# Superjomn/TiPS

Measured on AMD Instinct MI355X. Metric: device-resident fp32 bucket-sum GiB/s (% HBM peak); allreduce GiB/s 1/2/4/8 GPU, higher is better.
Workload: dtype f32

## Files before the change

### tips_amd/csrc/neg_protocol.cc

```cpp
#include "neg_protocol.h"

namespace tips {
namespace rt {

void put_announce_record(Writer& w, int type, int root, bool bad, int dtype, int64_t count,
                         const std::vector<int64_t>& shape, const std::string& name) {
  w.put<int32_t>(type);
  w.put<int32_t>(root);
  w.put<uint8_t>(bad ? 1 : 0);
  w.put<int32_t>(dtype);
  w.put<int64_t>(count);
  w.put<uint32_t>((uint32_t)shape.size());
  for (int64_t d : shape) w.put<int64_t>(d);
  w.str(name);
}
void get_announce_record(Reader& rd, Announce& a) {
  a.shape.clear();
  a.type = rd.get<int32_t>();
  a.root = rd.get<int32_t>();
  a.bad = rd.get<uint8_t>() != 0;
  a.dtype = rd.get<int32_t>();
  a.count = rd.get<int64_t>();
  const uint32_t ndim = rd.get<uint32_t>();
  if (ndim > TIPS_MAX_DIMS) rd.ok = false;
  for (uint32_t d = 0; d < ndim && rd.ok; d++) a.shape.push_back(rd.get<int64_t>());
  rd.str_into(a.name);
}

void put_response_entry(Writer& w, bool ok, const std::string& name, const std::string& err, const int64_t* sizes,
                        uint32_t m, size_t stride) {
  w.put<uint8_t>(ok ? 1 : 0);
  w.str(name);
  w.str(ok ? std::string() : err);
  w.put<uint32_t>(m);
  for (uint32_t i = 0; i < m; i++) w.put<int64_t>(sizes[(size_t)i * stride]);
}
bool get_response(const std::string& resp, const ResponseCache& cache, bool* shutdown, std::vector<Decision>& ds,
                  size_t* nd, int64_t* ncached) {
  Reader rd(resp);
  *shutdown = rd.get<uint8_t>() != 0;
  const uint32_t n = rd.get<uint32_t>();
  *nd = 0;
  for (uint32_t i = 0; i < n && rd.ok; i++) {
    if (*nd == ds.size()) ds.emplace_back();
    Decision& d = ds[(*nd)++];
    const uint8_t tag = rd.get<uint8_t>();
    d.sizes.clear();
    d.err.clear();
    if (tag == kCachedOk) {
      const uint32_t id = rd.get<uint32_t>();
      if (!cache.live(id)) return false;
      d.ok = true;
      d.name.assign(cache.entries[id].name);
      ++*ncached;
      continue;
    }
    d.ok = tag != 0;
    rd.str_into(d.name);
    rd.str_into(d.err);
    const uint32_t m = rd.get<uint32_t>();
    for (uint32_t k = 0; k < m && rd.ok && k < (1u << 20); k++) d.sizes.push_back(rd.get<int64_t>());
  }
  return rd.ok;
}

std::string shape_str(const int64_t* rec) {
  std::string s = "[";
  for (int64_t d = 0; d < rec[2]; d++) s += (d ? "," : "") + std::to_string(rec[3 + d]);
  return s + "]";
}

int check_records(const int64_t* t, int p) {
  const int W = TIPS_REQUEST_WORDS;
  const int64_t* r0 = t;
  for (int i = 1; i < p; i++)
    if (t[i * W + 1] != r0[1])
      return fail(TIPS_ERR_MISMATCH, "Mismatch data types found: %lld vs %lld.", (long long)r0[1], (long long)t[i * W + 1]);
  for (int i = 1; i < p; i++)
    if (t[i * W + 0] != r0[0])
      return fail(TIPS_ERR_MISMATCH, "Mismatched operations found: %lld vs %lld.", (long long)r0[0], (long long)t[i * W]);
  for (int i = 0; i < p; i++)
    if (t[i * W + 2] < 0 || t[i * W + 2] > TIPS_MAX_DIMS) return fail(TIPS_ERR_INVALID_ARG, "bad ndim in request %d", i);
  if (r0[0] == TIPS_REQ_ALLREDUCE || r0[0] == TIPS_REQ_BROADCAST) {
    for (int i = 1; i < p; i++) {
      const int64_t* ri = t + i * W;
      bool same = ri[2] == r0[2];
      for (int64_t d = 0; same && d < r0[2]; d++) same = ri[3 + d] == r0[3 + d];
      if (!same)
        return fail(TIPS_ERR_MISMATCH, "Mismatched %s tensor shapes: %s vs %s",
                    r0[0] == TIPS_REQ_BROADCAST ? "broadcast" : "allreduce", shape_str(r0).c_str(), shape_str(ri).c_str());
    }
  } else if (r0[0] == TIPS_REQ_ALLGATHER) {
    if (r0[2] == 0) return fail(TIPS_ERR_MISMATCH, "An empty tensor found");
    for (int i = 1; i < p; i++) {
      const int64_t* ri = t + i * W;
      if (ri[2] != r0[2])
        return fail(TIPS_ERR_MISMATCH, "Mismatched allgather tensor shapes: rank %lld vs %lld", (long long)r0[2],
                    (long long)ri[2]);
      for (int64_t d = 1; d < r0[2]; d++)
        if (ri[3 + d] != r0[3 + d])
          return fail(TIPS_ERR_MISMATCH, "Mismatched allgather tensor shapes: %lld-th dimension %lld vs %lld",
                      (long long)d, (long long)r0[3 + d], (long long)ri[3 + d]);
    }
  } else {
    return fail(TIPS_ERR_INVALID_ARG, "Not supported request type: %lld", (long long)r0[0]);
  }
  return 0;
}

void Table::announce(int rank, const Announce& a) {
  auto it = rows.find(a.name);
  if (it == rows.end()) {
    if (!spare.empty()) {
      auto nh = std::move(spare.back());
      spare.pop_back();
      nh.key() = a.name;
      Row& r = nh.mapped();
      r.rec.assign((size_t)p * TIPS_REQUEST_WORDS, 0);
      r.seen.assign(p, 0);
      r.roots.assign(p, 0);
      r.nseen = 0;
      r.queued = false;
      r.dup.clear();
      r.bad.clear();
      it = rows.insert(std::move(nh)).position;
    } else {
      Row r;
      r.rec.assign((size_t)p * TIPS_REQUEST_WORDS, 0);
      r.seen.assign(p, 0);
      r.roots.assign(p, 0);
      it = rows.emplace(a.name, std::move(r)).first;
    }
  }
  Row& r = it->second;
  if (r.seen[rank]) {
    if (r.dup.empty()) r.dup = "rank " + std::to_string(rank) + " enqueued " + a.name + " twice";
  } else {
    r.seen[rank] = 1;
    r.nseen++;
    if (a.bad && r.bad.empty())
      r.bad = "named request " + a.name + ": one device and one host pointer on rank " + std::to_string(rank);
    int64_t* rec = &r.rec[(size_t)rank * TIPS_REQUEST_WORDS];
    rec[0] = a.type;
    rec[1] = a.dtype;
    r.roots[rank] = a.root;
    rec[2] = (int64_t)a.shape.size();
    for (size_t d = 0; d < a.shape.size(); d++) rec[3 + d] = a.shape[d];
  }
  if (!r.queued && (!r.dup.empty() || r.nseen == p)) {
    r.queued = true;
    if (nready < ready_q.size()) ready_q[nready] = a.name;
    else ready_q.push_back(a.name);
    nready++;
  }
}

uint32_t Table::write_ready(Writer& w) {
  const int W = TIPS_REQUEST_WORDS;
  for (size_t q = 0; q < nready; q++) {
    const std::string& name = ready_q[q];
    auto it = rows.find(name);
    Row& r = it->second;
    const std::string* err = &r.dup;
    std::string why;
    bool ok = false;
    if (r.dup.empty() && !r.bad.empty()) {
      err = &r.bad;
    } else if (r.dup.empty()) {
      ok = check_records(r.rec.data(), p) == 0;
      if (!ok) why = last_error();
      if (ok && r.rec[0] == TIPS_REQ_BROADCAST)
        for (int i = 1; i < p && ok; i++)
          if (r.roots[i] != r.roots[0]) {
            ok = false;
            why = "Mismatched broadcast root ranks: " + std::to_string(r.roots[0]) + " vs " + std::to_string(r.roots[i]);
          }
      err = &why;
    }
    put_response_entry(w, ok, name, *err, &r.rec[3], ok && r.rec[0] == TIPS_REQ_ALLGATHER ? (uint32_t)p : 0, W);
    if (spare.size() < 4096) spare.push_back(rows.extract(it));
    else rows.erase(it);
  }
  const uint32_t n = (uint32_t)nready;
  nready = 0;
  return n;
}

Announce ResponseCache::expand(uint32_t id) const {
  const Entry& e = entries[id];
  Announce a;
  a.type = TIPS_REQ_ALLREDUCE;
  a.dtype = e.dtype;
  a.count = e.count;
  a.shape = e.shape;
  a.name = e.name;
  return a;
}

void ResponseCache::note(const Decision& d, const ReqParams* r) {
  if (sync_name(d.name)) return;
  const int32_t id = lookup(d.name, std::hash<std::string>()(d.name));
  if (!d.ok || !r || r->type != TIPS_REQ_ALLREDUCE) {
    if (id >= 0) {
      entries[(size_t)id].live = false;
      ids.erase(look);
    }
    return;
  }
  if (id >= 0) {
    Entry& e = entries[(size_t)id];
    e.dtype = r->dtype;
    e.count = r->count;
    e.shape = r->shape;
    return;
  }
  if (entries.size() >= cap) return;
  ids.emplace(NameKey{std::hash<std::string>()(d.name), d.name}, (uint32_t)entries.size());
  entries.push_back(Entry{d.name, r->dtype, r->count, r->shape, true});
}

void Coordinator::to_table(int32_t id) {
  if ((size_t)id >= idst.size()) idst.resize(cache.entries.size());
  IdState& st = idst[(size_t)id];
  if (st.table) return;
  st.table = true;
  for (int q = 0; q < 64 && st.mask; q++)
    if (st.mask & (1ull << q)) {
      st.mask &= ~(1ull << q);
      table.announce(q, cache.expand((uint32_t)id));
    }
  st.n = 0;
}

int Coordinator::decide(const std::string* all, std::string* resp) {
  bool everyone_stops = true;
  for (int r = 0; r < p; r++) {
    Reader rd(all[r]);
    bool stops;
    uint32_t n;
    get_announce_head(rd, &stops, &n);
    everyone_stops &= stops;
    for (uint32_t i = 0; i < n && rd.ok; i++) {
      get_announce_record(rd, a);
      if (!rd.ok) break;
      if (!cache.ids.empty()) {
        const int32_t id = cache.lookup(a.name, std::hash<std::string>()(a.name));
        if (id >= 0) to_table(id);
      }
      table.announce(r, a);
    }
    const uint32_t k = rd.get<uint32_t>();
    for (uint32_t i = 0; i < k && rd.ok; i++) {
      const uint32_t id = rd.get<uint32_t>();
      if (!cache.live(id)) {
        rd.ok = false;
        break;
      }
      if (idst.size() < cache.entries.size()) idst.resize(cache.entries.size());
      IdState& st = idst[id];
      const uint64_t bit = 1ull << r;
      if (st.table || (st.mask & bit)) {
        to_table(id);
        table.announce(r, cache.expand(id));
        continue;
      }
      st.mask |= bit;
      if (++st.n == p) {
        st.mask = 0;
        st.n = 0;
        id_ready.push_back(id);
      }
    }
    if (!rd.ok) return r;
  }
  for (size_t q = 0; q < table.nready; q++) {
    const int32_t id = idst.empty() ? -1 : cache.lookup(table.ready_q[q], std::hash<std::string>()(table.ready_q[q]));
    if (id >= 0 && (size_t)id < idst.size()) idst[id].table = false;
  }
  Writer w;
  w.b.swap(*resp);
  w.b.clear();
  const size_t count_at = put_response_head(w, everyone_stops);
  uint32_t n = table.write_ready(w);
  for (uint32_t id : id_ready) put_response_cached(w, id);
  n += (uint32_t)id_ready.size();
  id_ready.clear();
  put_response_count(w, count_at, n);
  resp->swap(w.b);
  return -1;
}

}
}
```

### tips_amd/csrc/neg_protocol.h

```cpp
#pragma once

#include <stdint.h>
#include <string.h>

#include <algorithm>
#include <string>
#include <unordered_map>
#include <vector>

#include "../../include/tips_hip.h"
#include "err.h"

namespace tips {
namespace rt {

struct Writer {
  std::string b;
  template <class T>
  void put(T v) {
    b.append(reinterpret_cast<const char*>(&v), sizeof v);
  }
  void str(const std::string& s) {
    put<uint32_t>((uint32_t)s.size());
    b += s;
  }
};

struct Reader {
  const std::string& b;
  size_t off = 0;
  bool ok = true;
  explicit Reader(const std::string& s) : b(s) {}
  template <class T>
  T get() {
    T v{};
    if (off + sizeof v > b.size()) {
      ok = false;
      return v;
    }
    memcpy(&v, b.data() + off, sizeof v);
    off += sizeof v;
    return v;
  }
  std::string str() {
    std::string s;
    str_into(s);
    return s;
  }
  void str_into(std::string& s) {
    const uint32_t n = get<uint32_t>();
    if (!ok || off + n > b.size()) {
      ok = false;
      s.clear();
      return;
    }
    s.assign(b.data() + off, n);
    off += n;
  }
};

struct Announce {
  int type = TIPS_REQ_ALLREDUCE, root = 0;
  bool bad = false;
  int dtype;
  int64_t count;
  std::vector<int64_t> shape;
  std::string name;
};

struct Decision {
  bool ok;
  std::string name, err;
  std::vector<int64_t> sizes;
};

struct NameKey {
  uint64_t h;
  std::string s;
  bool operator==(const NameKey& o) const { return h == o.h && s == o.s; }
};
struct NameKeyHash {
  size_t operator()(const NameKey& k) const { return (size_t)k.h; }
};

inline bool sync_name(const std::string& name) { return name.compare(0, 6, "~sync.") == 0; }

constexpr uint8_t kCachedOk = 2;

inline void put_announce_head(Writer& w, bool shutdown, uint32_t nfull) {
  w.put<uint8_t>(shutdown ? 1 : 0);
  w.put<uint32_t>(nfull);
}
inline void get_announce_head(Reader& rd, bool* shutdown, uint32_t* nfull) {
  *shutdown = rd.get<uint8_t>() != 0;
  *nfull = rd.get<uint32_t>();
}
void put_announce_record(Writer& w, int type, int root, bool bad, int dtype, int64_t count,
                         const std::vector<int64_t>& shape, const std::string& name);
void get_announce_record(Reader& rd, Announce& a);
inline void put_announce_ids(Writer& w, const std::vector<uint32_t>& ids) {
  w.put<uint32_t>((uint32_t)ids.size());
  for (uint32_t id : ids) w.put<uint32_t>(id);
}

inline size_t put_response_head(Writer& w, bool shutdown) {
  w.put<uint8_t>(shutdown ? 1 : 0);
  w.put<uint32_t>(0);
  return w.b.size() - sizeof(uint32_t);
}
inline void put_response_count(Writer& w, size_t at, uint32_t n) { memcpy(&w.b[at], &n, sizeof n); }
void put_response_entry(Writer& w, bool ok, const std::string& name, const std::string& err, const int64_t* sizes,
                        uint32_t m, size_t stride);
inline void put_response_cached(Writer& w, uint32_t id) {
  w.put<uint8_t>(kCachedOk);
  w.put<uint32_t>(id);
}
struct ResponseCache;
bool get_response(const std::string& resp, const ResponseCache& cache, bool* shutdown, std::vector<Decision>& ds,
                  size_t* nd, int64_t* ncached);

int check_records(const int64_t* t, int p);
std::string shape_str(const int64_t* rec);

struct Table {
  struct Row {
    std::vector<int64_t> rec;
    std::vector<int> roots;
    std::vector<char> seen;
    int nseen = 0;
    bool queued = false;
    std::string dup;
    std::string bad;
  };
  int p = 1;
  std::unordered_map<std::string, Row> rows;
  std::vector<std::string> ready_q;
  size_t nready = 0;
  std::vector<std::unordered_map<std::string, Row>::node_type> spare;

  void announce(int rank, const Announce& a);
  uint32_t write_ready(Writer& w);
};

struct ReqParams {
  int type, dtype;
  int64_t count;
  const std::vector<int64_t>& shape;
};

struct ResponseCache {
  static constexpr size_t kCacheCap = 1 << 16;
  struct Entry {
    std::string name;
    int dtype;
    int64_t count;
    std::vector<int64_t> shape;
    bool live;
  };
  std::vector<Entry> entries;
  std::unordered_map<NameKey, uint32_t, NameKeyHash> ids;
  NameKey look{0, std::string()};
  const bool by_id;
  const size_t cap;
  explicit ResponseCache(int ranks, bool by_id = true, size_t cap = kCacheCap) : by_id(by_id && ranks <= 64), cap(cap) {}

  int32_t lookup(const std::string& name, uint64_t h) {
    look.h = h;
    look.s.assign(name);
    auto it = ids.find(look);
    return it == ids.end() ? -1 : (int32_t)it->second;
  }
  int32_t cached_id(const std::string& name, uint64_t hash, int type, int dtype, const std::vector<int64_t>& shape,
                    bool bad) {
    if (!by_id || type != TIPS_REQ_ALLREDUCE || bad || ids.empty()) return -1;
    const int32_t id = lookup(name, hash);
    if (id < 0) return -1;
    const Entry& e = entries[(size_t)id];
    return e.dtype == dtype && e.shape == shape ? id : -1;
  }
  bool live(uint32_t id) const { return id < entries.size() && entries[id].live; }
  Announce expand(uint32_t id) const;
  void note(const Decision& d, const ReqParams* r);
};

struct Coordinator {
  Coordinator(int ranks, ResponseCache& cache) : p(ranks), cache(cache) { table.p = ranks; }
  int decide(const std::string* all, std::string* resp);
  void to_table(int32_t id);

  struct IdState {
    uint64_t mask = 0;
    int n = 0;
    bool table = false;
  };
  const int p;
  ResponseCache& cache;
  Table table;
  std::vector<IdState> idst;
  std::vector<uint32_t> id_ready;
  Announce a;
};

struct ExpectSet {
  std::vector<uint64_t> want, prev, cur;
  size_t hits = 0;

  void admitted(uint64_t name_hash) {
    if (!want.empty() && std::binary_search(want.begin(), want.end(), name_hash)) hits++;
  }
  bool complete() const { return !want.empty() && hits == want.size(); }
  void roll_add(const std::string& name, uint64_t name_hash) {
    if (!sync_name(name)) cur.push_back(name_hash);
  }
  void roll() {
    if (!cur.empty() && !(hits == want.size() && cur.size() == want.size())) {
      want.assign(cur.begin(), cur.end());
      want.insert(want.end(), prev.begin(), prev.end());
      std::sort(want.begin(), want.end());
      want.erase(std::unique(want.begin(), want.end()), want.end());
    }
    if (!cur.empty()) prev.swap(cur);
    cur.clear();
    hits = 0;
  }
};

}
}
```

### tips_amd/csrc/negotiate.cc

```cpp
#include <algorithm>
#include <chrono>
#include <condition_variable>
#include <pthread.h>
#include <sched.h>
#include <sys/prctl.h>
#include <deque>
#include <memory>
#include <thread>

#include "neg_protocol.h"
#include "net.h"
#include "rt.h"

namespace tips {
namespace rt {
namespace {

using namespace tips::net;

struct GroupEv {
  hipEvent_t ev = nullptr;
  std::atomic<bool> done{false};
  ~GroupEv() {
    if (ev) (void)hipEventDestroy(ev);
  }
};

inline int64_t steady_ns() {
  return std::chrono::duration_cast<std::chrono::nanoseconds>(std::chrono::steady_clock::now().time_since_epoch()).count();
}

class AdaptiveMutex {
 public:
  AdaptiveMutex() {
    pthread_mutexattr_t a;
    pthread_mutexattr_init(&a);
    pthread_mutexattr_settype(&a, env_i64("TIPS_ADAPTIVE_LOCKS", 1) ? PTHREAD_MUTEX_ADAPTIVE_NP : PTHREAD_MUTEX_NORMAL);
    pthread_mutex_init(&m_, &a);
    pthread_mutexattr_destroy(&a);
  }
  ~AdaptiveMutex() { pthread_mutex_destroy(&m_); }
  AdaptiveMutex(const AdaptiveMutex&) = delete;
  AdaptiveMutex& operator=(const AdaptiveMutex&) = delete;
  void lock() { pthread_mutex_lock(&m_); }
  bool try_lock() { return pthread_mutex_trylock(&m_) == 0; }
  void unlock() { pthread_mutex_unlock(&m_); }

 private:
  pthread_mutex_t m_;
};

enum : int { kFailed = -1, kQueued = 0, kAnnounced = 1, kLaunched = 2 , kDone = 3  };

struct Req {
  int64_t handle = 0;
  std::string name;
  uint64_t name_hash = 0;
  const void* in = nullptr;
  void* out = nullptr;
  int64_t count = 0;
  std::vector<int64_t> shape;
  int dtype = 0;
  int type = TIPS_REQ_ALLREDUCE;
  int root = 0;
  tips_alloc_fn alloc = nullptr;
  void* actx = nullptr;
  int64_t* out_rows = nullptr;
  bool host = false;
  hipStream_t stream = nullptr;
  hipEvent_t ev = nullptr;
  std::shared_ptr<GroupEv> gev;
  int state = kQueued;
  bool resolved() const { return state >= kLaunched || state == kFailed; }
  int code = TIPS_ERR_MISMATCH;
  std::string err;
  std::function<int()> body;
  tips_done_fn cb = nullptr;
  void* cb_ctx = nullptr;
  bool cb_queued = false;
  bool cb_only = false;
  bool classify = false;
  std::string bad;
};

std::atomic<uint64_t> g_next_shard{0};
std::atomic<int64_t> g_next_handle{0};

thread_local bool tl_negotiation_thread = false;
std::atomic<int64_t> g_sync_direct{0};

struct PtrRanges {
  struct Range {
    uintptr_t lo, len;
  };
  std::vector<Range> r;
  size_t last = 0;
  bool is_device(const void* p) {
    const uintptr_t a = (uintptr_t)p;
    if (last < r.size() && a - r[last].lo < r[last].len) return true;
    for (size_t k = 0; k < r.size(); k++)
      if (a - r[k].lo < r[k].len) {
        last = k;
        return true;
      }
    if (!is_device_ptr(p)) return false;
    hipDeviceptr_t base = nullptr;
    size_t size = 0;
    if (hipMemGetAddressRange(&base, &size, (hipDeviceptr_t)p) == hipSuccess && size > 0) {
      r.push_back(Range{(uintptr_t)base, (uintptr_t)size});
      last = r.size() - 1;
    } else {
      (void)hipGetLastError();
    }
    return true;
  }
};

using NameMap = std::unordered_map<NameKey, std::shared_ptr<Req>, NameKeyHash>;
using HandleMap = std::unordered_map<int64_t, std::shared_ptr<Req>>;

struct ReqSpec {
  ReqSpec(const char* name, const int64_t* shape, int ndim, int dtype, const void* in = nullptr, void* out = nullptr,
          void* stream = nullptr)
      : name(name), in(in), out(out), shape(shape), ndim(ndim), dtype(dtype), stream((hipStream_t)stream) {}
  const char* name;
  const void* in;
  void* out;
  const int64_t* shape;
  int ndim, dtype;
  hipStream_t stream;
  int type = TIPS_REQ_ALLREDUCE;
  int root = 0;
  tips_alloc_fn alloc = nullptr;
  void* actx = nullptr;
  int64_t* out_rows = nullptr;
  std::function<int()> body;
  tips_done_fn cb = nullptr;
  void* cb_ctx = nullptr;
};

const char* const kNotRunning = "negotiation thread is not running";

bool cpu_list(const std::string& path, cpu_set_t* set) {
  FILE* f = fopen(path.c_str(), "r");
  if (!f) return false;
  char buf[4096] = {};
  const bool ok = fgets(buf, sizeof buf, f) != nullptr;
  fclose(f);
  if (!ok) return false;
  CPU_ZERO(set);
  int n = 0;
  for (char* q = buf; *q && *q != '\n';) {
    char* e = nullptr;
    const long a = strtol(q, &e, 10);
    if (e == q) break;
    long b = a;
    if (*e == '-') b = strtol(e + 1, &e, 10);
    for (long c = a; c <= b && c < CPU_SETSIZE; c++) CPU_SET((int)c, set), n++;
    q = *e == ',' ? e + 1 : e;
  }
  return n > 0;
}

bool neg_bind_set(int cpu, cpu_set_t* out) {
  const char* v = getenv("TIPS_NEG_BIND");
  if (!v || !*v) v = "l3";
  if (!strcmp(v, "0") || !strcmp(v, "off") || cpu < 0) return false;
  const std::string base = "/sys/devices/system/cpu/cpu" + std::to_string(cpu);
  cpu_set_t want;
  if (!strcmp(v, "l3")) {
    if (!cpu_list(base + "/cache/index3/shared_cpu_list", &want)) return false;
  } else if (!strcmp(v, "core")) {
    if (!cpu_list(base + "/topology/thread_siblings_list", &want)) return false;
  } else {
    return false;
  }
  cpu_set_t allowed = process_cpus();
  CPU_AND(out, &want, &allowed);
  return CPU_COUNT(out) > 0;
}

void neg_thread_setup(const char* name, int start_cpu) {
  (void)pthread_setname_np(pthread_self(), name);
  cpu_set_t set;
  if (neg_bind_set(start_cpu, &set)) (void)pthread_setaffinity_np(pthread_self(), sizeof set, &set);
}

class Negotiator {
 public:
  static constexpr int kPortTries = 16;
  static constexpr uint64_t kMagic = 0x30474e4553504954ull;
  static constexpr uint64_t kConfirm = 0x31474e4553504954ull;
  struct Hello {
    uint64_t magic, key;
    int32_t rank, size;
    int64_t sync_direct;
  };
  struct Ack {
    uint64_t magic, key;
  };

  int start(int rank, int size, const char* host, int port, bool dry_run, int timeout_s, uint64_t key = 0,
            int64_t sync_direct = 0) {
    rank_ = rank;
    size_ = size;
    dry_ = dry_run;
    timeout_ms_ = timeout_s * 1000;
    by_name_.reserve(4096);
    by_handle_.reserve(4096);
    std::string err;
    if (size > 1) {
      const auto deadline = std::chrono::steady_clock::now() + std::chrono::milliseconds(timeout_ms_);
      auto ms_left = [&] {
        const auto l = std::chrono::duration_cast<std::chrono::milliseconds>(deadline - std::chrono::steady_clock::now()).count();
        return l > 0 ? (int)l : 0;
      };
      if (rank == 0) {
        for (int k = 0; k < kPortTries && lfd_ < 0; k++) lfd_ = listen_on(port + k, size, &err);
        if (lfd_ < 0) return fail(TIPS_ERR_BOOTSTRAP, "negotiation: ports %d-%d: %s", port, port + kPortTries - 1, err.c_str());
        peers_.assign(size, -1);
        std::vector<int64_t> counts(size, sync_direct);
        for (int joined = 0; joined < size - 1;) {
          pollfd pfd{lfd_, POLLIN, 0};
          if (ms_left() <= 0 || ::poll(&pfd, 1, ms_left()) <= 0)
            return fail(TIPS_ERR_BOOTSTRAP, "negotiation: %d rank(s) did not connect", size - 1 - joined);
          int c = ::accept(lfd_, nullptr, nullptr);
          if (c < 0) continue;
          Hello h{};
          const Ack a{kMagic, key};
          uint64_t confirm = 0;
          if (!recv_all(c, &h, sizeof h, 2000) || h.magic != kMagic || h.key != key || h.size != size || h.rank <= 0 ||
              h.rank >= size || !send_all(c, &a, sizeof a)) {
            ::close(c);
            continue;
          }
          if (!recv_all(c, &confirm, sizeof confirm, 2000) || confirm != kConfirm) {
            unconfirmed_joins()++;
            ::close(c);
            continue;
          }
          set_nodelay(c);
          if (peers_[h.rank] >= 0) {
            ::close(peers_[h.rank]);
            joined--;
          }
          peers_[h.rank] = c;
          counts[h.rank] = h.sync_direct;
          joined++;
        }
        std::string verdict;
        for (int r = 1; r < size && verdict.empty(); r++)
          if (counts[r] != counts[0])
            verdict = "rank " + std::to_string(r) + " issued " + std::to_string(counts[r]) +
                      " synchronous collectives before the negotiation started, rank 0 issued " +
                      std::to_string(counts[0]) + ": the first named request must come at the same point of "
                      "the collective order on every rank";
        Writer w;
        w.put<uint8_t>(verdict.empty() ? 1 : 0);
        w.str(verdict);
        for (int r = 1; r < size; r++) (void)send_msg(peers_[r], w.b);
        if (!verdict.empty()) {
          close_all();
          return fail(TIPS_ERR_MISMATCH, "negotiation: %s", verdict.c_str());
        }
      } else {
        const Hello h{kMagic, key, rank, size, sync_direct};
        static std::atomic<int> drop_first{-1};
        if (drop_first.load() < 0) {
          const char* v = getenv("TIPS_TEST_DROP_FIRST_HELLO");
          int expect = -1;
          drop_first.compare_exchange_strong(expect, v ? atoi(v) : 0);
        }
        while (up_ < 0) {
          for (int k = 0; k < kPortTries && up_ < 0; k++) {
            sockaddr_in sa;
            if (!resolve(host, port + k, &sa)) return fail(TIPS_ERR_BOOTSTRAP, "negotiation: cannot resolve %s", host);
            const int fd = connect_peer(sa);
            if (fd < 0) continue;
            Ack a{};
            const uint64_t confirm = kConfirm;
            if (send_all(fd, &h, sizeof h) && drop_first.load() > 0) {
              drop_first--;
              ::close(fd);
              continue;
            }
            if (recv_all(fd, &a, sizeof a, 5000) && a.magic == kMagic && a.key == key &&
                send_all(fd, &confirm, sizeof confirm)) {
              set_nodelay(fd);
              up_ = fd;
            } else {
              ::close(fd);
            }
          }
          if (up_ >= 0) break;
          if (ms_left() <= 0)
            return fail(TIPS_ERR_BOOTSTRAP, "negotiation: rank %d could not reach rank 0 at %s:%d-%d", rank, host, port,
                        port + kPortTries - 1);
          std::this_thread::sleep_for(std::chrono::milliseconds(20));
        }
        std::string v;
        if (!recv_msg(up_, &v, std::max(ms_left(), 1000))) {
          close_all();
          return fail(TIPS_ERR_BOOTSTRAP, "negotiation: rank %d got no verdict from rank 0", rank);
        }
        Reader rd(v);
        const bool ok = rd.get<uint8_t>() != 0;
        const std::string msg = rd.str();
        if (!ok || !rd.ok) {
          close_all();
          return fail(TIPS_ERR_MISMATCH, "negotiation: %s", rd.ok ? msg.c_str() : "malformed verdict");
        }
      }
    }
    own_.reset(new LoopOwn(size, env_i64("TIPS_RESPONSE_CACHE", 1) != 0));
    lockfree_ = env_i64("TIPS_ENQUEUE_LOCKFREE", 1) != 0;
    running_ = true;
    accepting_.store(true, std::memory_order_release);
    start_cpu_ = sched_getcpu();
    thread_ = std::thread([this] {
      tl_negotiation_thread = true;
      neg_thread_setup("tips-neg", start_cpu_);
      loop();
    });
    return 0;
  }

  void close_all() {
    for (int& fd : peers_)
      if (fd >= 0) ::close(fd), fd = -1;
    if (up_ >= 0) ::close(up_);
    if (lfd_ >= 0) ::close(lfd_);
    up_ = lfd_ = -1;
  }

  struct Prepared {
    std::shared_ptr<Req> r;
    NameMap::node_type name_node;
    HandleMap::node_type handle_node;
  };

  int prepare(Prepared& p, ReqSpec& q, PtrRanges* pr = nullptr) {
    if (q.ndim < 0 || q.ndim > TIPS_MAX_DIMS) return fail(TIPS_ERR_INVALID_ARG, "bad ndim %d", q.ndim);
    if (q.type == TIPS_REQ_ALLGATHER && q.ndim < 1) return fail(TIPS_ERR_INVALID_ARG, "An empty tensor found");
    auto r = std::make_shared<Req>();
    r->body = std::move(q.body);
    r->name = q.name;
    r->name_hash = std::hash<std::string>()(r->name);
    r->type = q.type;
    r->root = q.root;
    r->alloc = q.alloc;
    r->actx = q.actx;
    r->out_rows = q.out_rows;
    r->in = q.in;
    r->out = q.out;
    r->count = 1;
    r->shape.reserve((size_t)std::max(q.ndim, 1));
    for (int d = 0; d < q.ndim; d++) {
      if (q.shape[d] < 0) return fail(TIPS_ERR_INVALID_ARG, "negative dimension");
      r->shape.push_back(q.shape[d]);
      r->count *= q.shape[d];
    }
    if (q.ndim == 0) r->shape.push_back(1);
    r->dtype = q.dtype;
    r->stream = q.stream;
    r->cb = q.cb;
    r->cb_ctx = q.cb_ctx;
    r->cb_only = q.cb != nullptr;
    if (!dry_ && !r->body && r->count > 0) {
      static const bool at_enqueue = env_i64("TIPS_CLASSIFY_AT_ENQUEUE", 0) != 0;
      PtrRanges one;
      if (!pr && at_enqueue) pr = &one;
      if (pr) {
        const bool din = pr->is_device(q.in), dout = q.type == TIPS_REQ_ALLGATHER ? din : pr->is_device(q.out);
        if (din != dout) return fail(TIPS_ERR_INVALID_ARG, "named request %s: one device and one host pointer", q.name);
        r->host = !din;
      } else {
        r->classify = true;
      }
    }
    {
      thread_local int64_t tl_next = 0, tl_end = 0;
      if (tl_next == tl_end) {
        tl_next = g_next_handle.fetch_add(256) + 1;
        tl_end = tl_next + 256;
      }
      r->handle = tl_next++;
    }
    thread_local NameMap name_scratch;
    thread_local HandleMap handle_scratch;
    name_scratch.emplace(NameKey{r->name_hash, r->name}, r);
    p.name_node = name_scratch.extract(name_scratch.begin());
    if (!q.cb) {
      handle_scratch.emplace(r->handle, r);
      p.handle_node = handle_scratch.extract(handle_scratch.begin());
    }
    p.r = std::move(r);
    return 0;
  }

  int64_t commit(Prepared& p) {
    const int64_t h = p.r->handle;
    std::string why;
    const int rc = admit_prepared(p, false, &why, [](int) {});
    return rc ? fail(rc, "%s", why.c_str()) : h;
  }

  template <class Lap>
  int admit_prepared(Prepared& p, bool handle_anyway, std::string* why, Lap lap) {
    int code = 0;
    if (!running_) {
      *why = kNotRunning;
      code = TIPS_ERR_NOT_INITIALIZED;
    } else if (!by_name_.insert(std::move(p.name_node)).inserted) {
      *why = "a request named " + p.r->name + " is already pending";
      code = TIPS_ERR_INVALID_ARG;
    }
    lap(1);
    if (p.handle_node && (code == 0 || handle_anyway)) by_handle_.insert(std::move(p.handle_node));
    lap(2);
    if (code == 0) admit(std::move(p.r));
    return code;
  }

  int64_t enqueue(ReqSpec& q) {
    const bool cb = q.cb != nullptr;
    Prepared p;
    TRY(prepare(p, q));
    if (cb && !waiter_started_.load(std::memory_order_acquire)) {
      std::lock_guard<AdaptiveMutex> l(m_);
      if (!running_ || waiter_stop_) return fail(TIPS_ERR_NOT_INITIALIZED, "%s", kNotRunning);
      start_waiter_locked();
    }
    if (!lockfree_) {
      std::unique_lock<AdaptiveMutex> l(m_);
      drain_locked();
      const int64_t h = commit(p);
      if (h > 0) {
        last_arrival_ns_.store(steady_ns(), std::memory_order_release);
        if (fresh_.size() == 1) cv_.notify_all();
      }
      return h;
    }
    if (!accepting_.load(std::memory_order_acquire)) return fail(TIPS_ERR_NOT_INITIALIZED, "%s", kNotRunning);
    const int64_t h = p.r->handle;
    static std::atomic<int64_t> gap_us{-1};
    int64_t gap = gap_us.load(std::memory_order_relaxed);
    if (gap < 0) gap_us.store(gap = std::max<int64_t>(0, env_i64("TIPS_TEST_ENQUEUE_GAP_US", 0)), std::memory_order_relaxed);
    if (gap > 0) std::this_thread::sleep_for(std::chrono::microseconds(gap));
    Pending* node = new Pending{std::move(p), nullptr};
    thread_local const int tl_shard = (int)(g_next_shard.fetch_add(1, std::memory_order_relaxed) % kShards);
    std::atomic<Pending*>& head = shards_[tl_shard].head;
    Pending* old = head.load(std::memory_order_relaxed);
    do {
      node->next = old;
    } while (!head.compare_exchange_weak(old, node, std::memory_order_seq_cst, std::memory_order_relaxed));
    const int64_t now = steady_ns();
    if (now - last_arrival_ns_.load(std::memory_order_relaxed) > 2000)
      last_arrival_ns_.store(now, std::memory_order_release);
    if (!old && idle_.load(std::memory_order_seq_cst)) {
      std::lock_guard<AdaptiveMutex> l(m_);
      cv_.notify_all();
    }
    if (!accepting_.load(std::memory_order_seq_cst)) reclaim_after_stop();
    return h;
  }

  void reclaim_after_stop() {
    std::vector<std::shared_ptr<Req>> orphans;
    {
      std::lock_guard<AdaptiveMutex> l(m_);
      drain_locked(waiter_stop_ ? &orphans : nullptr);
    }
    for (auto& r : orphans) r->cb(r->cb_ctx, r->code, r->err.c_str());
  }

  void start_waiter_locked() {
    if (!waiter_.joinable())
      waiter_ = std::thread([this] {
        neg_thread_setup("tips-done", start_cpu_);
        waiter_loop();
      });
    waiter_started_.store(true, std::memory_order_release);
  }

  int drain_locked(std::vector<std::shared_ptr<Req>>* orphans = nullptr) {
    Pending* heads[kShards];
    int m = 0;
    for (Shard& sh : shards_)
      if (Pending* h = sh.head.exchange(nullptr, std::memory_order_seq_cst)) heads[m++] = h;
    if (!m) return 0;
    int count = 0;
    int64_t t = adm_prof_ ? steady_ns() : 0;
    auto lap = [&](int k) {
      if (!adm_prof_) return;
      const int64_t u = steady_ns();
      adm_ns_[k] += u - t;
      t = u;
    };
    Pending* rev[kShards] = {};
    for (bool more = true; more;) {
      more = false;
      for (int k = 0; k < m; k++)
        if (Pending* h = heads[k]) {
          heads[k] = h->next;
          __builtin_prefetch(h->p.r.get(), 1);
          h->next = rev[k];
          rev[k] = h;
          more = true;
        }
    }
    lap(0);
    for (int k = 0; k < m; k++) {
      for (Pending* q = rev[k]; q;) {
        Pending* n = q->next;
        Prepared& p = q->p;
        Req& r = *p.r;
        std::string why;
        if (const int code = admit_prepared(p, true, &why, lap)) {
          r.state = kFailed;
          r.code = code;
          r.err = why;
          if (r.cb) {
            if (orphans) orphans->push_back(p.r);
            else queue_done(p.r);
          }
          cv_.notify_all();
        }
        lap(3);
        delete q;
        lap(4);
        q = n;
        count++;
      }
    }
    return count;
  }

  void admit(std::shared_ptr<Req>&& r) {
    expect_.admitted(r->name_hash);
    fresh_.push_back(std::move(r));
  }

  int enqueue_list(std::vector<Prepared>& ps, int64_t* handles, std::string* first_err) {
    int rc = 0;
    std::unique_lock<AdaptiveMutex> l(m_);
    drain_locked();
    bool any = false;
    for (size_t i = 0; i < ps.size(); i++) {
      if (!ps[i].r) continue;
      handles[i] = commit(ps[i]);
      if (handles[i] < 0 && rc == 0) {
        rc = (int)handles[i];
        *first_err = last_error();
      }
      any |= handles[i] > 0;
    }
    if (any) {
      last_arrival_ns_.store(steady_ns(), std::memory_order_release);
      cv_.notify_all();
    }
    return rc;
  }

  int poll(int64_t h, bool block, bool routed = false) {
    std::shared_ptr<Req> r;
    {
      std::unique_lock<AdaptiveMutex> l(m_);
      drain_locked();
      auto it = by_handle_.find(h);
      if (it == by_handle_.end()) return fail(TIPS_ERR_INVALID_ARG, "unknown request handle %lld", (long long)h);
      r = it->second;
      if (r->cb) return fail(TIPS_ERR_INVALID_ARG, "request %s completes through its callback (tips_on_done)", r->name.c_str());
      if (block) cv_.wait(l, [&] { return r->resolved(); });
      if (!r->resolved()) return 0;
    }
    int rc = 1;
    if (r->state == kFailed) {
      rc = fail(r->code, "%s", r->err.c_str());
    } else if (r->state == kLaunched && !routed && !event_done(*r)) {
      const hipError_t e = finish_event(*r, block);
      if (e == hipErrorNotReady) return 0;
      if (e != hipSuccess) rc = fail(TIPS_ERR_HIP, "request %s: %s", r->name.c_str(), hipGetErrorString(e));
    }
    HandleMap::node_type gone;
    {
      std::lock_guard<AdaptiveMutex> l(m_);
      gone = release_locked(*r);
    }
    return rc;
  }

  static bool event_done(const Req& r) { return r.gev && r.gev->done.load(std::memory_order_acquire); }
  static hipError_t finish_event(Req& r, bool block) {
    hipEvent_t ev = r.gev ? r.gev->ev : r.ev;
    const hipError_t e = block ? hipEventSynchronize(ev) : hipEventQuery(ev);
    if (e == hipSuccess && r.gev) r.gev->done.store(true, std::memory_order_release);
    return e;
  }

  HandleMap::node_type release_locked(Req& r) {
    if (r.ev) ev_pool_.push_back(r.ev);
    r.ev = nullptr;
    r.gev.reset();
    return r.cb_only ? HandleMap::node_type() : by_handle_.extract(r.handle);
  }

  int on_done(int64_t h, tips_done_fn fn, void* ctx) {
    std::lock_guard<AdaptiveMutex> l(m_);
    drain_locked();
    auto it = by_handle_.find(h);
    if (it == by_handle_.end()) return fail(TIPS_ERR_INVALID_ARG, "unknown request handle %lld", (long long)h);
    auto& r = it->second;
    if (r->cb) return fail(TIPS_ERR_INVALID_ARG, "request %s already has a completion callback", r->name.c_str());
    if (waiter_stop_) {
      fn(ctx, r->state == kFailed ? r->code : 0, r->state == kFailed ? r->err.c_str() : "");
      return 0;
    }
    r->cb = fn;
    r->cb_ctx = ctx;
    start_waiter_locked();
    if (r->resolved()) queue_done(r);
    return 0;
  }

  int stop() {
    {
      std::lock_guard<AdaptiveMutex> l(m_);
      if (!running_ && !thread_.joinable() && !waiter_.joinable()) return 0;
      want_stop_ = true;
      cv_.notify_all();
    }
    if (thread_.joinable()) thread_.join();
    {
      std::lock_guard<AdaptiveMutex> l(m_);
      accepting_.store(false, std::memory_order_seq_cst);
      drain_locked();
      waiter_stop_ = true;
      done_cv_.notify_all();
    }
    if (waiter_.joinable()) waiter_.join();
    close_all();
    peers_.clear();
    release_device_resources();
    return loop_err_.empty() ? 0 : fail(TIPS_ERR_BOOTSTRAP, "%s", loop_err_.c_str());
  }

  int64_t cached_decisions() const { return cached_decisions_.load(std::memory_order_relaxed); }

  int64_t callbacks_called() {
    std::lock_guard<AdaptiveMutex> l(m_);
    return cb_called_;
  }

  void release_device_resources() {
    std::vector<hipEvent_t> evs;
    {
      std::lock_guard<AdaptiveMutex> l(m_);
      evs.swap(ev_pool_);
    }
    for (hipEvent_t e : evs) (void)hipEventDestroy(e);
    join_ev_.release();
    if (neg_stream_) (void)hipStreamDestroy(neg_stream_);
    neg_stream_ = nullptr;
  }

  ~Negotiator() {
    {
      std::lock_guard<AdaptiveMutex> l(m_);
      waiter_stop_ = true;
      done_cv_.notify_all();
    }
    if (waiter_.joinable()) waiter_.join();
    std::vector<std::shared_ptr<Req>> orphans;
    {
      std::lock_guard<AdaptiveMutex> l(m_);
      running_ = false;
      drain_locked(&orphans);
    }
    for (auto& r : orphans) r->cb(r->cb_ctx, r->code, r->err.c_str());
    for (auto& kv : by_handle_)
      if (kv.second->ev) ev_pool_.push_back(kv.second->ev);
    release_device_resources();
  }

  bool running() {
    std::lock_guard<AdaptiveMutex> l(m_);
    return running_;
  }
  std::vector<std::string> log() {
    std::lock_guard<AdaptiveMutex> l(m_);
    return log_;
  }
  void note(const std::string& s) {
    std::lock_guard<AdaptiveMutex> l(m_);
    log_.push_back(s);
  }

 private:
  void loop() {
    (void)prctl(PR_SET_TIMERSLACK, (unsigned long)std::max<int64_t>(1, env_i64("TIPS_NEG_TIMER_SLACK_NS", 1000)), 0, 0, 0);
    const auto cycle = std::chrono::microseconds(std::max<int64_t>(50, env_i64("TIPS_CYCLE_TIME_US", 1000)));
    const auto linger = std::chrono::microseconds(std::max<int64_t>(0, env_i64("TIPS_BATCH_LINGER_US", 30)));
    const bool spin_linger = env_i64("TIPS_LINGER_SPIN", 0) != 0;
    const bool expect_on = env_i64("TIPS_LINGER_EXPECT", 1) != 0;
    const int64_t expect_quiet_ns = 1000 * std::max<int64_t>(0, env_i64("TIPS_LINGER_EXPECT_US", 4));
    const int64_t expect_step_ns = 8000;
    auto complete = [&] { return expect_on && expect_.complete(); };
    const bool trace = env_i64("TIPS_NEG_TRACE", 0) != 0;
    {
      std::lock_guard<AdaptiveMutex> l(m_);
      adm_prof_ = trace;
    }
    auto us_since = [](std::chrono::steady_clock::time_point t) {
      return (long long)std::chrono::duration_cast<std::chrono::microseconds>(std::chrono::steady_clock::now() - t).count();
    };
    Writer w;
    std::string resp;
    std::vector<Decision> ds;
    std::vector<uint32_t> cids;
    std::vector<Req*> full;
    ResponseCache& cache = own_->cache;
    while (true) {
      std::vector<std::shared_ptr<Req>> batch;
      bool stopping;
      set_phase("waiting for requests");
      long long t_linger = 0, t_tail = 0;
      int windows = 0, last_drained = 0;
      int64_t drain_ns = 0, last_drain_ns = 0, wait_ns = 0;
      auto timed_drain = [&] {
        const int64_t a = steady_ns();
        last_drained = drain_locked();
        last_drain_ns = steady_ns() - a;
        drain_ns += last_drain_ns;
      };
      {
        std::unique_lock<AdaptiveMutex> l(m_);
        idle_.store(true, std::memory_order_seq_cst);
        cv_.wait_for(l, cycle, [&] {
          return !fresh_.empty() || any_pending() || want_stop_;
        });
        idle_.store(false, std::memory_order_relaxed);
        drain_locked();
        const auto t0 = std::chrono::steady_clock::now();
        windows = 0;
        if (!fresh_.empty() && !want_stop_ && linger.count() > 0) {
          const int64_t start = steady_ns(), linger_ns = (int64_t)linger.count() * 1000,
                        cycle_ns = (int64_t)cycle.count() * 1000;
          while (!want_stop_) {
            timed_drain();
            const int64_t now = steady_ns(), quiet = now - last_arrival_ns_.load(std::memory_order_acquire);
            const bool done = complete();
            const int64_t need = done ? std::min(expect_quiet_ns, linger_ns) : linger_ns;
            if (quiet >= need || now - start >= cycle_ns) break;
            windows++;
            if (spin_linger) {
              l.unlock();
              const int64_t stop_at = std::min(now + linger_ns, start + cycle_ns);
              for (int64_t t = steady_ns(); t < stop_at; t = steady_ns()) {
                if (t - last_arrival_ns_.load(std::memory_order_acquire) >= linger_ns) break;
                __builtin_ia32_pause();
              }
              l.lock();
            } else {
              int64_t wait = std::min(need - quiet, cycle_ns - (now - start));
              if (expect_on && !expect_.want.empty() && !done) wait = std::min(wait, expect_step_ns);
              const int64_t a = steady_ns();
              cv_.wait_for(l, std::chrono::nanoseconds(wait));
              wait_ns += steady_ns() - a;
            }
          }
        }
        timed_drain();
        batch.assign(fresh_.begin(), fresh_.end());
        fresh_.clear();
        if (expect_on) {
          for (auto& r : batch) expect_.roll_add(r->name, r->name_hash);
          expect_.roll();
        }
        for (auto& r : batch) r->state = kAnnounced;
        stopping = want_stop_;
        t_linger = us_since(t0);
        t_tail = (steady_ns() - last_arrival_ns_.load(std::memory_order_acquire)) / 1000;
      }
      for (auto& r : batch)
        if (r->classify) {
          const bool din = is_device_ptr(r->in), dout = r->type == TIPS_REQ_ALLGATHER ? din : is_device_ptr(r->out);
          if (din != dout) r->bad = "one device and one host pointer";
          r->host = !din;
          r->classify = false;
        }
      const auto t_x = std::chrono::steady_clock::now();
      w.b.clear();
      cids.clear();
      full.clear();
      for (auto& r : batch) {
        const int32_t id = cache.cached_id(r->name, r->name_hash, r->type, r->dtype, r->shape, !r->bad.empty());
        if (id >= 0) cids.push_back((uint32_t)id);
        else full.push_back(r.get());
      }
      put_announce_head(w, stopping, (uint32_t)full.size());
      for (Req* r : full) put_announce_record(w, r->type, r->root, !r->bad.empty(), r->dtype, r->count, r->shape, r->name);
      put_announce_ids(w, cids);
      set_phase("exchange (cycle " + std::to_string((long long)cycles_) + ", announcing " + std::to_string(batch.size()) + ")");
      if (!exchange(w.b, &resp)) break;
      {
        std::lock_guard<std::mutex> l(phase_mu_);
        cycles_++;
      }
      bool shutdown = false;
      size_t nd = 0;
      int64_t ncached = 0;
      const bool wellformed = get_response(resp, cache, &shutdown, ds, &nd, &ncached);
      cached_decisions_.fetch_add(ncached, std::memory_order_relaxed);
      if (!wellformed) {
        set_loop_error("negotiation: malformed response");
        break;
      }
      const long long t_exchange = us_since(t_x);
      const auto t_e = std::chrono::steady_clock::now();
      execute(ds, nd);
      if (trace && (!batch.empty() || nd))
        fprintf(stderr, "[tips neg] rank %d cycle %lld: announced %zu, decided %zu; linger %lld us (%d windows, "
                "ended %lld us after the latest arrival; waits %lld us, admissions %lld us, the last %d in %lld us), exchange %lld us "
                "(rank 0's decision %lld us), execute %lld us\n", rank_, (long long)cycles_, batch.size(), nd, t_linger, windows,
                t_tail, (long long)(wait_ns / 1000), (long long)(drain_ns / 1000), last_drained, (long long)(last_drain_ns / 1000),
                t_exchange, (long long)(rank_ == 0 ? own_->decide_ns / 1000 : -1), us_since(t_e));
      if (trace && (!batch.empty() || nd)) {
        std::lock_guard<AdaptiveMutex> l(m_);
        fprintf(stderr, "[tips neg]   admission phases (us): walk %lld, name table %lld, handle table %lld, queue %lld, "
                "free %lld\n", (long long)(adm_ns_[0] / 1000), (long long)(adm_ns_[1] / 1000), (long long)(adm_ns_[2] / 1000),
                (long long)(adm_ns_[3] / 1000), (long long)(adm_ns_[4] / 1000));
        for (int64_t& x : adm_ns_) x = 0;
      }
      if (shutdown) break;
    }
    std::lock_guard<AdaptiveMutex> l(m_);
    accepting_.store(false, std::memory_order_seq_cst);
    drain_locked();
    running_ = false;
    std::vector<std::string> unmatched;
    for (auto& kv : by_name_) unmatched.push_back(kv.first.s);
    std::sort(unmatched.begin(), unmatched.end());
    for (auto& name : unmatched) {
      auto& r = by_name_.find(NameKey{std::hash<std::string>()(name), name})->second;
      r->state = kFailed;
      r->code = TIPS_ERR_MISMATCH;
      r->err = "request " + name + " was not enqueued on every rank before shutdown";
      if (dry_) log_.push_back(name + " ERR " + r->err);
      if (r->cb) queue_done(r);
    }
    by_name_.clear();
    cv_.notify_all();
  }

  void queue_done(const std::shared_ptr<Req>& r) {
    if (r->cb_queued) return;
    r->cb_queued = true;
    done_q_.push_back(r);
    done_cv_.notify_all();
  }

  void waiter_loop() {
    std::deque<std::shared_ptr<Req>> batch;
    while (true) {
      {
        std::unique_lock<AdaptiveMutex> l(m_);
        done_cv_.wait(l, [&] { return !done_q_.empty() || waiter_stop_; });
        if (done_q_.empty()) return;
        batch.swap(done_q_);
      }
      for (auto& r : batch) {
        int status = 0;
        std::string msg;
        if (r->state == kFailed) {
          status = r->code;
          msg = r->err;
        } else if (r->state == kLaunched && !event_done(*r)) {
          set_waiter_req(r, true);
          const hipError_t e = finish_event(*r, true);
          if (e != hipSuccess) {
            status = TIPS_ERR_HIP;
            msg = std::string("request ") + r->name + ": " + hipGetErrorString(e);
          }
        }
        set_waiter_req(r, false);
        r->cb(r->cb_ctx, status, msg.c_str());
      }
      set_waiter_req(nullptr, false);
      std::vector<HandleMap::node_type> gone;
      gone.reserve(batch.size());
      {
        std::lock_guard<AdaptiveMutex> l(m_);
        for (auto& r : batch) gone.push_back(release_locked(*r));
        cb_called_ += (int64_t)batch.size();
      }
      gone.clear();
      batch.clear();
    }
  }

  bool exchange(const std::string& mine, std::string* resp) {
    if (size_ == 1) return decide(&mine, resp);
    if (rank_ != 0) {
      if (!send_msg(up_, mine) || !recv_msg(up_, resp, timeout_ms_)) {
        set_loop_error("negotiation: lost rank 0");
        return false;
      }
      return true;
    }
    std::vector<std::string> all(size_);
    all[0] = mine;
    for (int r = 1; r < size_; r++)
      if (!recv_msg(peers_[r], &all[r], timeout_ms_)) {
        set_loop_error("negotiation: lost rank " + std::to_string(r));
        return false;
      }
    if (!decide(all.data(), resp)) return false;
    for (int r = 1; r < size_; r++)
      if (!send_msg(peers_[r], *resp)) {
        set_loop_error("negotiation: lost rank " + std::to_string(r));
        return false;
      }
    return true;
  }

  bool decide(const std::string* all, std::string* resp) {
    const int64_t a = steady_ns();
    const int bad_rank = own_->coord.decide(all, resp);
    own_->decide_ns = steady_ns() - a;
    if (bad_rank >= 0) set_loop_error("negotiation: malformed announce from rank " + std::to_string(bad_rank));
    return bad_rank < 0;
  }

  void execute(const std::vector<Decision>& ds, size_t n) {
    std::vector<std::shared_ptr<Req>> reqs(n);
    std::vector<NameMap::node_type> gone;
    gone.reserve(n);
    {
      std::lock_guard<AdaptiveMutex> l(m_);
      for (size_t i = 0; i < n; i++) {
        look_.h = std::hash<std::string>()(ds[i].name);
        look_.s.assign(ds[i].name);
        auto it = by_name_.find(look_);
        if (it == by_name_.end()) continue;
        reqs[i] = it->second;
        gone.push_back(by_name_.extract(it));
        if (dry_) {
          std::string sz;
          for (size_t k = 0; k < ds[i].sizes.size(); k++) sz += (k ? "," : " sizes=") + std::to_string(ds[i].sizes[k]);
          log_.push_back(ds[i].name + (ds[i].ok ? " OK" + sz : " ERR " + ds[i].err));
        }
      }
    }
    gone.clear();
    for (size_t i = 0; i < n; i++) {
      if (const Req* r = reqs[i].get()) {
        const ReqParams rp{r->type, r->dtype, r->count, r->shape};
        own_->cache.note(ds[i], &rp);
      } else {
        own_->cache.note(ds[i], nullptr);
      }
    }
    std::vector<int> state(n, 0), code(n, TIPS_ERR_MISMATCH);
    std::vector<std::string> msg(n);
    for (size_t i = 0; i < n; i++) {
      state[i] = ds[i].ok ? (dry_ ? kDone : kLaunched) : kFailed;
      msg[i] = ds[i].err;
    }
    auto failed = [&](size_t k, int rc) {
      state[k] = kFailed;
      code[k] = rc;
      msg[k] = last_error();
    };
    if (!dry_) {
      State& st = S();
      const bool fuse = env_i64("TIPS_NEGOTIATED_FUSION", 1) != 0;
      const int64_t threshold = fusion_threshold_bytes();
      auto joins = [&](size_t k, bool host, int dtype) {
        return reqs[k] && state[k] == kLaunched && !reqs[k]->body && reqs[k]->type == TIPS_REQ_ALLREDUCE &&
               reqs[k]->host == host && reqs[k]->dtype == dtype;
      };
      for (size_t i = 0; i < n;) {
        if (!reqs[i] || state[i] != kLaunched) {
          i++;
          continue;
        }
        {
          std::lock_guard<std::mutex> l(phase_mu_);
          executed_++;
          exec_i_ = i;
          exec_n_ = n;
          exec_req_ = reqs[i];
        }
        if (reqs[i]->body) {
          const int rc = reqs[i]->body();
          if (rc != 0) failed(i, rc);
          else state[i] = kDone;
          i++;
          continue;
        }
        const int dtype = reqs[i]->dtype;
        if (reqs[i]->type == TIPS_REQ_ALLREDUCE && reqs[i]->host && fuse) {
          size_t j = i;
          while (j < n && joins(j, true, dtype)) j++;
          if (j - i >= 2) {
            std::vector<BatchItem> items;
            for (size_t k = i; k < j; k++) items.push_back(BatchItem{reqs[k]->in, reqs[k]->out, reqs[k]->count});
            int rc;
            {
              std::lock_guard<std::mutex> lk(st.mu);
              rc = set_device(st);
              if (rc == 0) rc = fused_allreduce_host(st, items.data(), (int)items.size(), dtype, nullptr);
            }
            for (size_t k = i; k < j; k++) {
              if (rc != 0) failed(k, rc);
              else state[k] = kDone;
            }
            i = j;
            continue;
          }
        }
        if (reqs[i]->type != TIPS_REQ_ALLREDUCE || reqs[i]->host) {
          const int rc = run_other(*reqs[i], ds[i].sizes);
          if (rc != 0) failed(i, rc);
          else if (reqs[i]->host) state[i] = kDone;
          i++;
          continue;
        }
        std::lock_guard<std::mutex> lk(st.mu);
        const int rc0 = set_device(st);
        const int64_t es = tips::dtype_size(dtype);
        size_t j = i;
        int64_t bytes = 0;
        while (fuse && j < n && joins(j, false, dtype) && reqs[j]->count * es < threshold &&
               round_up(bytes, kAlignBytes) + reqs[j]->count * es <= threshold) {
          bytes = round_up(bytes, kAlignBytes) + reqs[j]->count * es;
          j++;
        }
        int rc = rc0;
        if (j - i >= 2) {
          if (rc == 0) rc = run_batch(st, reqs, i, j);
        } else {
          j = i + 1;
          auto& r = reqs[i];
          if (rc == 0) rc = allreduce_device(st, r->in, r->out, r->count, r->dtype, r->stream);
          if (rc == 0) rc = take_event(*r);
          if (rc == 0 && hipEventRecord(r->ev, r->stream) != hipSuccess) rc = fail(TIPS_ERR_HIP, "hipEventRecord failed");
        }
        if (rc != 0)
          for (size_t k = i; k < j; k++) failed(k, rc);
        i = j;
      }
    }
    std::lock_guard<AdaptiveMutex> l(m_);
    for (size_t i = 0; i < n; i++)
      if (reqs[i]) {
        reqs[i]->state = state[i];
        reqs[i]->code = code[i];
        reqs[i]->err = msg[i];
        if (reqs[i]->cb) queue_done(reqs[i]);
      }
    cv_.notify_all();
  }

  int take_event(Req& r) {
    {
      std::lock_guard<AdaptiveMutex> l(m_);
      if (!ev_pool_.empty()) {
        r.ev = ev_pool_.back();
        ev_pool_.pop_back();
        return 0;
      }
    }
    TRY(set_device(S()));
    HIP_TRY(hipEventCreateWithFlags(&r.ev, hipEventDisableTiming));
    return 0;
  }

  int run_other(Req& r, const std::vector<int64_t>& sizes) {
    if (r.type == TIPS_REQ_ALLREDUCE) {
      TRY(tips_allreduce(r.in, r.out, r.count, r.dtype, TIPS_OP_SUM, r.stream));
    } else if (r.type == TIPS_REQ_BROADCAST) {
      TRY(tips_broadcast(r.in, r.out, r.count, r.dtype, r.root, r.stream));
    } else {
      const int64_t es = tips::dtype_size(r.dtype);
      int64_t row = 1, rows = 0;
      for (size_t d = 1; d < r.shape.size(); d++) row *= r.shape[d];
      std::vector<int64_t> counts;
      for (int64_t v : sizes) {
        counts.push_back(v * row);
        rows += v;
      }
      if ((int)counts.size() != S().size) return fail(TIPS_ERR_MISMATCH, "allgather %s: sizes of %zu ranks", r.name.c_str(), counts.size());
      const int64_t bytes = rows * row * es;
      std::string why;
      if (bytes > 0) {
        if (!r.alloc) why = "no output allocator";
        else if (!(r.out = r.alloc(r.actx, bytes))) why = "the output allocator returned NULL for " + std::to_string(bytes) + " B";
      }
      const int64_t mine = why.empty() ? 1 : 0;
      std::vector<int64_t> all((size_t)S().size, 1);
      TRY(tips_allgather_i64(&mine, 1, all.data()));
      if (!why.empty()) return fail(TIPS_ERR_HIP, "allgather %s: %s", r.name.c_str(), why.c_str());
      for (int q = 0; q < S().size; q++)
        if (!all[q]) return fail(TIPS_ERR_HIP, "allgather %s: rank %d could not allocate its output", r.name.c_str(), q);
      if (r.out_rows) *r.out_rows = rows;
      TRY(tips_allgatherv(r.in, r.count, r.out, counts.data(), r.dtype, r.stream));
    }
    if (!r.host) {
      TRY(take_event(r));
      HIP_TRY(hipEventRecord(r.ev, r.stream));
    }
    return 0;
  }

  int run_batch(State& st, std::vector<std::shared_ptr<Req>>& reqs, size_t i, size_t j) {
    std::vector<hipStream_t> streams;
    for (size_t k = i; k < j; k++)
      if (std::find(streams.begin(), streams.end(), reqs[k]->stream) == streams.end()) streams.push_back(reqs[k]->stream);
    hipStream_t s = streams[0];
    if (streams.size() > 1) {
      if (!neg_stream_) HIP_TRY(hipStreamCreateWithFlags(&neg_stream_, hipStreamNonBlocking));
      s = neg_stream_;
      TRY(join_ev_.ensure(streams.size()));
      for (size_t k = 0; k < streams.size(); k++) TRY(join(s, streams[k], join_ev_.ev[k]));
    }
    std::vector<BatchItem> items;
    items.reserve(j - i);
    for (size_t k = i; k < j; k++) items.push_back(BatchItem{reqs[k]->in, reqs[k]->out, reqs[k]->count});
    TRY(fused_allreduce(st, items.data(), (int)items.size(), reqs[i]->dtype, s));
    auto g = std::make_shared<GroupEv>();
    HIP_TRY(hipEventCreateWithFlags(&g->ev, hipEventDisableTiming));
    HIP_TRY(hipEventRecord(g->ev, s));
    if (streams.size() > 1)
      for (hipStream_t u : streams) HIP_TRY(hipStreamWaitEvent(u, g->ev, 0));
    for (size_t k = i; k < j; k++) reqs[k]->gev = g;
    return 0;
  }

  void set_loop_error(const std::string& e) {
    std::lock_guard<AdaptiveMutex> l(m_);
    if (loop_err_.empty()) loop_err_ = e;
  }

  int rank_ = 0, size_ = 1, timeout_ms_ = 600000;
  bool dry_ = false;
  int lfd_ = -1, up_ = -1;
  std::vector<int> peers_;
  struct LoopOwn {
    ResponseCache cache;
    Coordinator coord;
    int64_t decide_ns = 0;
    LoopOwn(int size, bool by_id) : cache(size, by_id), coord(size, cache) {}
  };
  std::unique_ptr<LoopOwn> own_;
  std::thread thread_;
  AdaptiveMutex m_;
  std::condition_variable_any cv_;
  bool running_ = false, want_stop_ = false;
  std::atomic<bool> accepting_{false};
  struct Pending {
    Prepared p;
    Pending* next = nullptr;
  };
  static constexpr int kShards = 8;
  struct alignas(64) Shard {
    std::atomic<Pending*> head{nullptr};
  };
  Shard shards_[kShards];
  bool any_pending() {
    for (Shard& sh : shards_)
      if (sh.head.load(std::memory_order_seq_cst)) return true;
    return false;
  }
  std::atomic<bool> idle_{false};
  bool lockfree_ = true;
  std::atomic<bool> waiter_started_{false};
  std::deque<std::shared_ptr<Req>> fresh_;
  ExpectSet expect_;
  bool adm_prof_ = false;
  int64_t adm_ns_[5] = {};
  std::atomic<int64_t> last_arrival_ns_{0};
  NameMap by_name_;
  NameKey look_{0, std::string()};
  std::atomic<int64_t> cached_decisions_{0};
  HandleMap by_handle_;
  std::vector<std::string> log_;
  std::vector<hipEvent_t> ev_pool_;
  std::string loop_err_;
  hipStream_t neg_stream_ = nullptr;
  std::thread waiter_;
  int start_cpu_ = -1;
  std::deque<std::shared_ptr<Req>> done_q_;
  std::condition_variable_any done_cv_;
  bool waiter_stop_ = false;
  int64_t cb_called_ = 0;

  EventPool join_ev_;

  std::mutex phase_mu_;
  std::string phase_ = "start";
  std::shared_ptr<Req> waiter_req_;
  bool waiter_syncing_ = false;
  int64_t cycles_ = 0, executed_ = 0;
  size_t exec_i_ = 0, exec_n_ = 0;
  std::shared_ptr<Req> exec_req_;
  void set_phase(std::string p) {
    std::lock_guard<std::mutex> l(phase_mu_);
    phase_ = std::move(p);
    exec_req_.reset();
  }
  void set_waiter_req(const std::shared_ptr<Req>& r, bool syncing) {
    std::lock_guard<std::mutex> l(phase_mu_);
    waiter_req_ = r;
    waiter_syncing_ = syncing;
  }

 public:
  std::atomic<int64_t> sync_seq{0};

  std::string debug_state() {
    std::string out;
    {
      std::lock_guard<std::mutex> l(phase_mu_);
      std::string ph = phase_;
      if (exec_req_) {
        const Req& r = *exec_req_;
        ph = "execute " + std::to_string(exec_i_) + "/" + std::to_string(exec_n_) + ": " + r.name +
             (r.body ? " (routed call)" : r.host ? " (host)" : r.type != TIPS_REQ_ALLREDUCE ? " (other)" : "");
      }
      out = "rank " + std::to_string(rank_) + " cycles " + std::to_string((long long)cycles_) + " executed " +
            std::to_string((long long)executed_) + " | negotiation: " + ph + " | completion: " +
            (!waiter_req_ ? std::string("idle")
                          : waiter_syncing_ ? "hipEventSynchronize of " + waiter_req_->name + (waiter_req_->gev ? " (fused batch)" : "")
                                            : "callback of " + waiter_req_->name);
    }
    std::unique_lock<AdaptiveMutex> l(m_, std::try_to_lock);
    if (!l.owns_lock()) return out + " | (request lock held)";
    out += " | fresh " + std::to_string(fresh_.size()) + " pending " + std::to_string(by_name_.size()) + " handles " +
           std::to_string(by_handle_.size()) + " done_q " + std::to_string(done_q_.size()) + " callbacks " +
           std::to_string((long long)cb_called_);
    int k = 0;
    for (auto& kv : by_name_) {
      if (k++ == 8) break;
      out += (k == 1 ? " | waiting for other ranks: " : ", ") + kv.first.s + "(state " + std::to_string(kv.second->state) + ")";
    }
    if (!done_q_.empty()) out += " | next callback: " + done_q_.front()->name + "(state " + std::to_string(done_q_.front()->state) + ")";
    return out;
  }
};

AdaptiveMutex g_neg_mu;
std::shared_ptr<Negotiator> g_neg;
std::atomic<uint64_t> g_neg_gen{0};
std::string g_neg_failed;
Negotiator* g_selftest_neg = nullptr;

int negotiation_port() {
  return (int)env_i64("TIPS_NEGOTIATION_PORT", env_i64("MASTER_PORT", 29500) + 19);
}

const char* master_addr() {
  const char* h = getenv("MASTER_ADDR");
  return (h && *h) ? h : "127.0.0.1";
}

}

bool on_negotiation_thread() { return tl_negotiation_thread; }

bool negotiation_running() {
  std::shared_ptr<Negotiator> n;
  {
    std::lock_guard<AdaptiveMutex> l(g_neg_mu);
    n = g_neg;
  }
  return n && n->running();
}

int negotiation_stop() {
  std::shared_ptr<Negotiator> n;
  {
    std::lock_guard<AdaptiveMutex> l(g_neg_mu);
    n.swap(g_neg);
    g_neg_gen.fetch_add(1, std::memory_order_release);
    g_neg_failed.clear();
  }
  g_sync_direct = 0;
  return n ? n->stop() : 0;
}

bool route_collective(int type, int dtype, const int64_t* shape, int ndim, int root, const std::function<int()>& body,
                      int* rc) {
  if (tl_negotiation_thread) return false;
  std::shared_ptr<Negotiator> n;
  {
    std::lock_guard<AdaptiveMutex> l(g_neg_mu);
    n = g_neg;
  }
  if (!n || !n->running()) {
    State& st = S();
    if (st.initialized && st.size > 1) g_sync_direct++;
    return false;
  }
  const std::string name = "~sync." + std::to_string((long long)n->sync_seq++);
  ReqSpec q(name.c_str(), shape, ndim, dtype);
  q.type = type;
  q.root = root;
  q.body = body;
  const int64_t h = n->enqueue(q);
  if (h < 0) {
    *rc = (int)h;
    return true;
  }
  const int w = n->poll(h, true, true);
  *rc = w == 1 ? 0 : w;
  return true;
}

}
}

using namespace tips::rt;


namespace {

std::shared_ptr<Negotiator> negotiator(int* code) {
  std::lock_guard<AdaptiveMutex> l(g_neg_mu);
  if (!g_neg) {
    if (!g_neg_failed.empty()) {
      *code = fail(TIPS_ERR_MISMATCH, "%s", g_neg_failed.c_str());
      return nullptr;
    }
    State& st = S();
    int rank, size;
    uint64_t key;
    {
      std::lock_guard<std::mutex> lk(st.mu);
      if (!st.initialized) {
        *code = fail(TIPS_ERR_NOT_INITIALIZED, "tips_init has not been called");
        return nullptr;
      }
      rank = st.rank;
      size = st.size;
      key = st.peer_key;
    }
    auto neg = std::make_shared<Negotiator>();
    const int rc = neg->start(rank, size, master_addr(), negotiation_port(), false,
                              (int)env_i64("TIPS_NEGOTIATION_TIMEOUT", 600), key, g_sync_direct.load());
    if (rc) {
      *code = rc;
      if (rc == TIPS_ERR_MISMATCH) g_neg_failed = last_error();
      return nullptr;
    }
    g_neg = std::move(neg);
    g_neg_gen.fetch_add(1, std::memory_order_release);
  }
  return g_neg;
}

std::shared_ptr<Negotiator> current() {
  std::lock_guard<AdaptiveMutex> l(g_neg_mu);
  return g_neg;
}

Negotiator* cached(bool create, int* code) {
  thread_local std::shared_ptr<Negotiator> tl;
  thread_local uint64_t tl_gen = ~0ull;
  const uint64_t g = g_neg_gen.load(std::memory_order_acquire);
  if (g == tl_gen && tl) return tl.get();
  tl = create ? negotiator(code) : current();
  tl_gen = g;
  return tl.get();
}

Negotiator* started() {
  int code = 0;
  Negotiator* n = cached(false, &code);
  if (!n) fail(TIPS_ERR_NOT_INITIALIZED, "no named request was ever enqueued");
  return n;
}

int check_named(const char* name, const void* in, void* out, const int64_t* shape, int ndim, int dtype, int type,
                int root, tips_alloc_fn alloc) {
  TRY(check_dtype(dtype));
  if (!name || !*name || ndim < 0 || ndim > TIPS_MAX_DIMS || (ndim > 0 && !shape))
    return fail(TIPS_ERR_INVALID_ARG, "bad named request");
  int64_t count = 1;
  for (int d = 0; d < ndim; d++) count *= shape[d] < 0 ? 0 : shape[d];
  if (count > 0 && (!in || (type != TIPS_REQ_ALLGATHER && !out))) return fail(TIPS_ERR_INVALID_ARG, "bad named request");
  if (type == TIPS_REQ_ALLGATHER && !alloc) return fail(TIPS_ERR_INVALID_ARG, "named allgather needs an output allocator");
  if (type == TIPS_REQ_BROADCAST) {
    const int size = tips_size();
    if (root < 0 || (size > 0 && root >= size)) return fail(TIPS_ERR_INVALID_ARG, "root rank %d out of range", root);
  }
  return 0;
}

int64_t enqueue_named(const char* name, const void* in, void* out, const int64_t* shape, int ndim, int dtype,
                      void* stream, int type = TIPS_REQ_ALLREDUCE, int root = 0, tips_alloc_fn alloc = nullptr,
                      void* actx = nullptr, int64_t* out_rows = nullptr) {
  TRY(check_named(name, in, out, shape, ndim, dtype, type, root, alloc));
  int code = TIPS_ERR_NOT_INITIALIZED;
  Negotiator* n = cached(true, &code);
  if (!n) return code;
  ReqSpec q(name, shape, ndim, dtype, in, out, stream);
  q.type = type;
  q.root = root;
  q.alloc = alloc;
  q.actx = actx;
  q.out_rows = out_rows;
  return n->enqueue(q);
}

template <class Dims>
int enqueue_named_list(const char* const* names, const void* const* ins, void* const* outs, int n, int dtype,
                       void* stream, int64_t* handles, Dims dims) {
  int rc = 0;
  std::string first_err;
  auto refused = [&](int i, int code) {
    handles[i] = code;
    if (rc == 0) {
      rc = code;
      first_err = last_error();
    }
  };
  int code = TIPS_ERR_NOT_INITIALIZED;
  std::shared_ptr<Negotiator> neg;
  std::vector<Negotiator::Prepared> ps((size_t)n);
  PtrRanges pr;
  for (int i = 0; i < n; i++) {
    const std::pair<const int64_t*, int> d = dims(i);
    int e = d.second == -2 ? (int)TIPS_ERR_INVALID_ARG
            : d.second < 0 ? fail(TIPS_ERR_INVALID_ARG, "bad named allreduce request")
                           : check_named(names[i], ins[i], outs[i], d.first, d.second, dtype, TIPS_REQ_ALLREDUCE, 0, nullptr);
    if (e == 0 && !neg && !(neg = negotiator(&code))) e = code;
    if (e == 0) {
      ReqSpec q(names[i], d.first, d.second, dtype, ins[i], outs[i], stream);
      e = neg->prepare(ps[(size_t)i], q, &pr);
    }
    if (e) refused(i, e);
  }
  if (neg && env_i64("TIPS_LIST_ONE_LOCK", 1) == 0) {
    std::vector<Negotiator::Prepared> one(1);
    for (int i = 0; i < n; i++) {
      if (!ps[(size_t)i].r) continue;
      one[0] = std::move(ps[(size_t)i]);
      std::string err;
      const int e = neg->enqueue_list(one, handles + i, &err);
      if (e && rc == 0) {
        rc = e;
        first_err = err;
      }
    }
  } else if (neg) {
    std::string err;
    const int e = neg->enqueue_list(ps, handles, &err);
    if (e && rc == 0) {
      rc = e;
      first_err = err;
    }
  }
  return rc ? fail(rc, "%s", first_err.c_str()) : 0;
}


}

extern "C" {

int64_t tips_enqueue_allreduce(const char* name, const void* in, void* out, int64_t count, int dtype, void* stream) {
  if (count < 0) return fail(TIPS_ERR_INVALID_ARG, "bad named allreduce request");
  return enqueue_named(name, in, out, &count, 1, dtype, stream);
}

int64_t tips_enqueue_allreduce_shaped(const char* name, const void* in, void* out, const int64_t* shape, int ndim,
                                      int dtype, void* stream) {
  return enqueue_named(name, in, out, shape, ndim, dtype, stream);
}

int64_t tips_enqueue_broadcast(const char* name, const void* in, void* out, const int64_t* shape, int ndim,
                               int dtype, int root, void* stream) {
  return enqueue_named(name, in, out, shape, ndim, dtype, stream, TIPS_REQ_BROADCAST, root);
}

int64_t tips_enqueue_allgather(const char* name, const void* in, const int64_t* shape, int ndim, int dtype,
                               void* stream, tips_alloc_fn alloc, void* ctx, int64_t* out_rows) {
  return enqueue_named(name, in, nullptr, shape, ndim, dtype, stream, TIPS_REQ_ALLGATHER, 0, alloc, ctx, out_rows);
}


int tips_poll(int64_t handle) {
  Negotiator* n = started();
  if (!n) return TIPS_ERR_NOT_INITIALIZED;
  return n->poll(handle, false);
}

int tips_wait(int64_t handle) {
  Negotiator* n = started();
  if (!n) return TIPS_ERR_NOT_INITIALIZED;
  const int rc = n->poll(handle, true);
  return rc == 1 ? 0 : rc;
}

int64_t tips_enqueue_allreduce_cb(const char* name, const void* in, void* out, const int64_t* shape, int ndim, int dtype,
                                  void* stream, tips_done_fn fn, void* ctx) {
  if (!fn) return fail(TIPS_ERR_INVALID_ARG, "null completion callback");
  TRY(check_named(name, in, out, shape, ndim, dtype, TIPS_REQ_ALLREDUCE, 0, nullptr));
  int code = TIPS_ERR_NOT_INITIALIZED;
  Negotiator* n = cached(true, &code);
  if (!n) return code;
  ReqSpec q(name, shape, ndim, dtype, in, out, stream);
  q.cb = fn;
  q.cb_ctx = ctx;
  return n->enqueue(q);
}

int tips_on_done(int64_t handle, tips_done_fn fn, void* ctx) {
  if (!fn) return fail(TIPS_ERR_INVALID_ARG, "null completion callback");
  Negotiator* n = started();
  if (!n) return TIPS_ERR_NOT_INITIALIZED;
  return n->on_done(handle, fn, ctx);
}

int tips_debug_state(char* out, int64_t cap) {
  if (!out || cap < 1) return fail(TIPS_ERR_INVALID_ARG, "tips_debug_state: no buffer");
  std::string st = "no negotiation";
  std::unique_lock<AdaptiveMutex> l(g_neg_mu, std::try_to_lock);
  if (!l.owns_lock()) st = "(negotiation being started or stopped)";
  else if (g_neg) st = g_neg->debug_state();
  else if (g_selftest_neg) st = g_selftest_neg->debug_state();
  snprintf(out, (size_t)cap, "%s", st.c_str());
  return 0;
}

int tips_net_stats(int64_t* self_connects_refused, int64_t* unconfirmed_joins_refused) {
  if (self_connects_refused) *self_connects_refused = tips::net::self_connects().load();
  if (unconfirmed_joins_refused) *unconfirmed_joins_refused = tips::net::unconfirmed_joins().load();
  return 0;
}

int tips_enqueue_allreduce_n(const char* const* names, const void* const* ins, void* const* outs, const int64_t* counts,
                             int n, int dtype, void* stream, int64_t* handles) {
  if (n < 0 || (n > 0 && (!names || !ins || !outs || !counts || !handles)))
    return fail(TIPS_ERR_INVALID_ARG, "bad named allreduce list");
  return enqueue_named_list(names, ins, outs, n, dtype, stream, handles, [&](int i) {
    return std::make_pair(&counts[i], counts[i] < 0 ? -1 : 1);
  });
}

int tips_enqueue_allreduce_shaped_n(const char* const* names, const void* const* ins, void* const* outs,
                                    const int* ndims, const int64_t* dims, int n, int dtype, void* stream,
                                    int64_t* handles) {
  if (n < 0 || (n > 0 && (!names || !ins || !outs || !ndims || !handles)))
    return fail(TIPS_ERR_INVALID_ARG, "bad named allreduce list");
  std::vector<int64_t> offs((size_t)n + 1, 0);
  for (int i = 0; i < n; i++) offs[(size_t)i + 1] = offs[(size_t)i] + (ndims[i] > 0 && ndims[i] <= TIPS_MAX_DIMS ? ndims[i] : 0);
  return enqueue_named_list(names, ins, outs, n, dtype, stream, handles, [&](int i) {
    const bool ok = ndims[i] >= 0 && ndims[i] <= TIPS_MAX_DIMS && (ndims[i] == 0 || dims);
    if (!ok) fail(TIPS_ERR_INVALID_ARG, "bad ndim %d for %s", ndims[i], names[i] ? names[i] : "?");
    return std::make_pair(dims ? dims + offs[(size_t)i] : (const int64_t*)nullptr, ok ? ndims[i] : -2);
  });
}

int tips_wait_n(const int64_t* handles, int n) {
  if (n < 0 || (n > 0 && !handles)) return fail(TIPS_ERR_INVALID_ARG, "bad handle list");
  int rc = 0;
  std::string first_err;
  for (int i = 0; i < n; i++) {
    if (handles[i] <= 0) continue;
    const int w = tips_wait(handles[i]);
    if (w < 0 && rc == 0) {
      rc = w;
      first_err = last_error();
    }
  }
  return rc ? fail(rc, "%s", first_err.c_str()) : 0;
}

#ifdef TIPS_DEV
namespace {

struct SelftestCount {
  std::atomic<int64_t> done{0};
};

void selftest_done(void* ctx, int status, const char* message) {
  (void)status;
  (void)message;
  static_cast<SelftestCount*>(ctx)->done++;
}

}

int tips_negotiation_selftest(int rank, int size, const char* host, int port, const char* requests, char* out,
                              int64_t cap) {
  if (size < 1 || rank < 0 || rank >= size || !requests || !out || cap < 1)
    return fail(TIPS_ERR_INVALID_ARG, "bad selftest args");
  std::vector<std::vector<std::string>> per(1);
  int64_t synccount = 0;
  for (const char* p = requests; *p;) {
    const char* e = strchr(p, '\n');
    std::string line(p, e ? (size_t)(e - p) : strlen(p));
    p = e ? e + 1 : p + line.size();
    if (line.empty()) continue;
    if (line.rfind("@synccount ", 0) == 0) {
      synccount = atoll(line.c_str() + 11);
      continue;
    }
    size_t k = 0;
    if (line[0] == 't' && line.find(':') != std::string::npos && isdigit((unsigned char)line[1])) {
      k = (size_t)atoi(line.c_str() + 1);
      line = line.substr(line.find(':') + 1);
      while (!line.empty() && line[0] == ' ') line.erase(0, 1);
      if (k > 64) return fail(TIPS_ERR_INVALID_ARG, "selftest: thread %zu", k);
    }
    if (per.size() <= k) per.resize(k + 1);
    per[k].push_back(line);
  }
  const bool cbs = per.size() > 1;
  Negotiator neg;
  TRY(neg.start(rank, size, (host && *host) ? host : "127.0.0.1", port, true, 120, 0, synccount));
  struct Registered {
    explicit Registered(Negotiator* n) {
      std::lock_guard<AdaptiveMutex> l(g_neg_mu);
      g_selftest_neg = n;
    }
    ~Registered() {
      std::lock_guard<AdaptiveMutex> l(g_neg_mu);
      g_selftest_neg = nullptr;
    }
  } registered(&neg);
  const auto t0 = std::chrono::steady_clock::now();
  std::vector<SelftestCount> counts(per.size());
  std::vector<int> issued(per.size(), 0), rcs(per.size(), 0);
  auto run = [&](size_t k) {
    std::vector<int64_t> handles;
    bool batching = false;
    std::vector<Negotiator::Prepared> batch;
    auto issued_one = [&](int64_t h) -> bool {
      if (h < 0) {
        rcs[k] = (int)h;
        return false;
      }
      if (cbs) {
        issued[k]++;
        if (neg.on_done(h, selftest_done, &counts[k]) != 0) {
          rcs[k] = TIPS_ERR_INVALID_ARG;
          return false;
        }
      } else {
        handles.push_back(h);
      }
      return true;
    };
    for (const std::string& line : per[k]) {
      char nm[256], dims[256] = "", kind[64] = "ar";
      long long dt = 0, cnt = 0;
      if (line == "@batch") {
        batching = true;
        batch.clear();
      } else if (line == "@endbatch") {
        batching = false;
        std::vector<int64_t> hs(batch.size(), 0);
        std::string err;
        if (neg.enqueue_list(batch, hs.data(), &err) != 0) {
          rcs[k] = TIPS_ERR_INVALID_ARG;
          return;
        }
        for (int64_t h : hs)
          if (!issued_one(h)) return;
      } else if (line.rfind("@sleep ", 0) == 0) {
        std::this_thread::sleep_for(std::chrono::milliseconds(atoi(line.c_str() + 7)));
      } else if (line == "@wait") {
        if (cbs) {
          while (counts[k].done.load() < issued[k]) std::this_thread::sleep_for(std::chrono::milliseconds(1));
        } else {
          for (int64_t h : handles) (void)neg.poll(h, true);
          handles.clear();
        }
      } else if (line == "@mark") {
        const auto us = std::chrono::duration_cast<std::chrono::microseconds>(std::chrono::steady_clock::now() - t0);
        neg.note("# mark " + std::to_string((long long)us.count()));
      } else if (sscanf(line.c_str(), "%255s %lld %lld %255s %63s", nm, &dt, &cnt, dims, kind) >= 3) {
        std::vector<int64_t> shape;
        if (strcmp(dims, "-") == 0) dims[0] = 0;
        const int type = strncmp(kind, "ag", 2) == 0 ? TIPS_REQ_ALLGATHER : strncmp(kind, "bc", 2) == 0 ? TIPS_REQ_BROADCAST
                                                                                                    : TIPS_REQ_ALLREDUCE;
        const int root = (type == TIPS_REQ_BROADCAST && kind[2] == ':') ? atoi(kind + 3) : 0;
        for (const char* q = dims; *q;) {
          shape.push_back(strtoll(q, nullptr, 10));
          q = strchr(q, ',');
          q = q ? q + 1 : "";
        }
        if (shape.empty()) shape.push_back(cnt);
        ReqSpec q(nm, shape.data(), (int)shape.size(), (int)dt);
        q.type = type;
        q.root = root;
        if (batching) {
          batch.emplace_back();
          if (neg.prepare(batch.back(), q) != 0) {
            rcs[k] = TIPS_ERR_INVALID_ARG;
            return;
          }
        } else if (!issued_one(neg.enqueue(q))) {
          return;
        }
      }
    }
    if (!cbs)
      for (int64_t h : handles) (void)neg.poll(h, false);
  };
  std::vector<std::thread> threads;
  for (size_t k = 1; k < per.size(); k++) threads.emplace_back(run, k);
  run(0);
  for (auto& t : threads) t.join();
  const int rc = neg.stop();
  for (int r : rcs)
    if (r) return r;
  std::string log;
  for (auto& l : neg.log()) log += l + "\n";
  log += "# cached decisions " + std::to_string((long long)neg.cached_decisions()) + "\n";
  if (cbs) {
    int64_t n = 0;
    for (auto& c : counts) n += c.done.load();
    log += "callbacks " + std::to_string((long long)n) + "\n";
  }
  snprintf(out, (size_t)cap, "%s", log.c_str());
  return rc;
}

int tips_negotiation_stop_race_selftest(int threads, int per_thread, int stop_after_us, int rounds, int port,
                                        int64_t* result) {
  if (threads < 1 || per_thread < 1 || rounds < 1 || !result) return fail(TIPS_ERR_INVALID_ARG, "bad args");
  for (int k = 0; k < 4; k++) result[k] = 0;
  struct Slot {
    std::atomic<int> calls{0};
    bool accepted = false;
  };
  auto count_cb = [](void* ctx, int, const char*) { static_cast<Slot*>(ctx)->calls.fetch_add(1); };
  for (int round = 0; round < rounds; round++) {
    std::vector<Slot> slots((size_t)threads * per_thread);
    {
      Negotiator neg;
      TRY(neg.start(0, 1, "127.0.0.1", port, true, 30, 0, 0));
      std::atomic<bool> go{false};
      std::vector<std::thread> th;
      for (int t = 0; t < threads; t++)
        th.emplace_back([&, t] {
          while (!go.load()) std::this_thread::yield();
          const int64_t shape[1] = {4};
          for (int i = 0; i < per_thread; i++) {
            Slot& sl = slots[(size_t)t * per_thread + i];
            const std::string name = "r" + std::to_string(round) + "/t" + std::to_string(t) + "/" + std::to_string(i);
            ReqSpec q(name.c_str(), shape, 1, TIPS_FLOAT32);
            q.cb = count_cb;
            q.cb_ctx = &sl;
            const int64_t h = neg.enqueue(q);
            sl.accepted = h > 0;
          }
        });
      go.store(true);
      std::this_thread::sleep_for(std::chrono::microseconds(stop_after_us));
      (void)neg.stop();
      for (auto& x : th) x.join();
      for (auto& sl : slots) {
        const int c = sl.calls.load();
        result[0] += sl.accepted;
        result[1] += c;
        result[2] += sl.accepted ? c != 1 : c != 0;
        result[3] += !sl.accepted;
      }
    }
  }
  return result[2] == 0 ? TIPS_OK : fail(TIPS_ERR_MISMATCH, "%lld requests saw a wrong number of callbacks", (long long)result[2]);
}
#endif

}
```

Measured before the change: 6282.

## Pool intrusive-refcounted requests, batch wait_n under one lock, skip cached names

Replaces shared_ptr-managed requests with an intrusive refcounted Req recycled through a lock-free free list, reusing its map nodes across enqueues. The separate Pending wrapper allocation goes away, and cached decisions can carry an id instead of copying the name. tips_wait_n now waits on all handles under one lock and releases them together, instead of calling tips_wait once per handle. This is meant to cut host-side allocation and locking on the negotiation path. In exchange it adds more complex lifetime management and a risk of use-after-recycle bugs.

```diff
diff --git a/tips_amd/csrc/neg_protocol.cc b/tips_amd/csrc/neg_protocol.cc
--- a/tips_amd/csrc/neg_protocol.cc
+++ b/tips_amd/csrc/neg_protocol.cc
@@ -36,7 +36,7 @@
   for (uint32_t i = 0; i < m; i++) w.put<int64_t>(sizes[(size_t)i * stride]);
 }
 bool get_response(const std::string& resp, const ResponseCache& cache, bool* shutdown, std::vector<Decision>& ds,
-                  size_t* nd, int64_t* ncached) {
+                  size_t* nd, int64_t* ncached, bool cached_names) {
   Reader rd(resp);
   *shutdown = rd.get<uint8_t>() != 0;
   const uint32_t n = rd.get<uint32_t>();
@@ -47,11 +47,14 @@
     const uint8_t tag = rd.get<uint8_t>();
     d.sizes.clear();
     d.err.clear();
+    d.id = -1;
     if (tag == kCachedOk) {
       const uint32_t id = rd.get<uint32_t>();
       if (!cache.live(id)) return false;
       d.ok = true;
-      d.name.assign(cache.entries[id].name);
+      d.id = (int32_t)id;
+      if (cached_names) d.name.assign(cache.entries[id].name);
+      else d.name.clear();
       ++*ncached;
       continue;
     }
@@ -219,6 +222,15 @@
   entries.push_back(Entry{d.name, r->dtype, r->count, r->shape, true});
 }
 
+void ResponseCache::drop(uint32_t id) {
+  if (!live(id)) return;
+  Entry& e = entries[id];
+  e.live = false;
+  look.h = std::hash<std::string>()(e.name);
+  look.s.assign(e.name);
+  ids.erase(look);
+}
+
 void Coordinator::to_table(int32_t id) {
   if ((size_t)id >= idst.size()) idst.resize(cache.entries.size());
   IdState& st = idst[(size_t)id];
diff --git a/tips_amd/csrc/neg_protocol.h b/tips_amd/csrc/neg_protocol.h
--- a/tips_amd/csrc/neg_protocol.h
+++ b/tips_amd/csrc/neg_protocol.h
@@ -72,6 +72,7 @@
   bool ok;
   std::string name, err;
   std::vector<int64_t> sizes;
+  int32_t id = -1;
 };
 
 struct NameKey {
@@ -117,7 +118,7 @@
 }
 struct ResponseCache;
 bool get_response(const std::string& resp, const ResponseCache& cache, bool* shutdown, std::vector<Decision>& ds,
-                  size_t* nd, int64_t* ncached);
+                  size_t* nd, int64_t* ncached, bool cached_names = true);
 
 int check_records(const int64_t* t, int p);
 std::string shape_str(const int64_t* rec);
@@ -181,6 +182,7 @@
   bool live(uint32_t id) const { return id < entries.size() && entries[id].live; }
   Announce expand(uint32_t id) const;
   void note(const Decision& d, const ReqParams* r);
+  void drop(uint32_t id);
 };
 
 struct Coordinator {
diff --git a/tips_amd/csrc/negotiate.cc b/tips_amd/csrc/negotiate.cc
--- a/tips_amd/csrc/negotiate.cc
+++ b/tips_amd/csrc/negotiate.cc
@@ -30,6 +30,13 @@
   return std::chrono::duration_cast<std::chrono::nanoseconds>(std::chrono::steady_clock::now().time_since_epoch()).count();
 }
 
+inline bool neg_trace() {
+  static std::atomic<int> on{-1};
+  int v = on.load(std::memory_order_relaxed);
+  if (v < 0) on.store(v = env_i64("TIPS_NEG_TRACE", 0) != 0 ? 1 : 0, std::memory_order_relaxed);
+  return v != 0;
+}
+
 class AdaptiveMutex {
  public:
   AdaptiveMutex() {
@@ -52,7 +59,23 @@
 
 enum : int { kFailed = -1, kQueued = 0, kAnnounced = 1, kLaunched = 2 , kDone = 3  };
 
+struct Req;
+class Negotiator;
+using NameMap = std::unordered_map<NameKey, Req*, NameKeyHash>;
+using HandleMap = std::unordered_map<int64_t, Req*>;
+
 struct Req {
+  std::atomic<int> refs{0};
+  Negotiator* owner = nullptr;
+  std::atomic<Req*> pool_next{nullptr};
+  Req* next = nullptr;
+  NameMap::node_type name_node;
+  HandleMap::node_type handle_node;
+  NameMap::iterator name_it;
+  uint64_t name_epoch = 0;
+  int32_t cid = -1;
+  bool listed = false;
+
   int64_t handle = 0;
   std::string name;
   uint64_t name_hash = 0;
@@ -81,6 +104,75 @@
   bool cb_only = false;
   bool classify = false;
   std::string bad;
+
+  void reset() {
+    next = nullptr;
+    cid = -1;
+    listed = false;
+    handle = 0;
+    in = nullptr;
+    out = nullptr;
+    count = 0;
+    dtype = 0;
+    type = TIPS_REQ_ALLREDUCE;
+    root = 0;
+    alloc = nullptr;
+    actx = nullptr;
+    out_rows = nullptr;
+    host = false;
+    stream = nullptr;
+    ev = nullptr;
+    gev.reset();
+    state = kQueued;
+    code = TIPS_ERR_MISMATCH;
+    err.clear();
+    body = nullptr;
+    cb = nullptr;
+    cb_ctx = nullptr;
+    cb_queued = false;
+    cb_only = false;
+    classify = false;
+    bad.clear();
+  }
+};
+
+void req_unreferenced(Req* r);
+
+class ReqPtr {
+ public:
+  ReqPtr() = default;
+  explicit ReqPtr(Req* p) : p_(p) {
+    if (p_) p_->refs.fetch_add(1, std::memory_order_relaxed);
+  }
+  ReqPtr(const ReqPtr& o) : ReqPtr(o.p_) {}
+  ReqPtr(ReqPtr&& o) noexcept : p_(o.p_) { o.p_ = nullptr; }
+  ReqPtr& operator=(ReqPtr o) noexcept {
+    std::swap(p_, o.p_);
+    return *this;
+  }
+  ~ReqPtr() { reset(); }
+  void reset() {
+    Req* q = p_;
+    p_ = nullptr;
+    if (q && q->refs.fetch_sub(1, std::memory_order_acq_rel) == 1) req_unreferenced(q);
+  }
+  static ReqPtr adopt(Req* p) {
+    ReqPtr r;
+    r.p_ = p;
+    return r;
+  }
+  Req* detach() {
+    Req* q = p_;
+    p_ = nullptr;
+    return q;
+  }
+  Req* get() const { return p_; }
+  Req* operator->() const { return p_; }
+  Req& operator*() const { return *p_; }
+  explicit operator bool() const { return p_ != nullptr; }
+
+ private:
+  Req* p_ = nullptr;
 };
 
 std::atomic<uint64_t> g_next_shard{0};
@@ -115,9 +207,6 @@
     return true;
   }
 };
-
-using NameMap = std::unordered_map<NameKey, std::shared_ptr<Req>, NameKeyHash>;
-using HandleMap = std::unordered_map<int64_t, std::shared_ptr<Req>>;
 
 struct ReqSpec {
   ReqSpec(const char* name, const int64_t* shape, int ndim, int dtype, const void* in = nullptr, void* out = nullptr,
@@ -208,6 +297,7 @@
     timeout_ms_ = timeout_s * 1000;
     by_name_.reserve(4096);
     by_handle_.reserve(4096);
+    name_buckets_ = by_name_.bucket_count();
     std::string err;
     if (size > 1) {
       const auto deadline = std::chrono::steady_clock::now() + std::chrono::milliseconds(timeout_ms_);
@@ -334,17 +424,59 @@
   }
 
   struct Prepared {
-    std::shared_ptr<Req> r;
-    NameMap::node_type name_node;
-    HandleMap::node_type handle_node;
+    ReqPtr r;
   };
+
+  ReqPtr take() {
+    while (pop_busy_.test_and_set(std::memory_order_acquire)) __builtin_ia32_pause();
+    Req* r = free_head_.load(std::memory_order_acquire);
+    while (r && !free_head_.compare_exchange_weak(r, r->pool_next.load(std::memory_order_relaxed),
+                                                  std::memory_order_acquire, std::memory_order_acquire)) {
+    }
+    pop_busy_.clear(std::memory_order_release);
+    if (r) {
+      pool_reused_.fetch_add(1, std::memory_order_relaxed);
+      r->reset();
+    } else {
+      r = new Req();
+      r->owner = this;
+      pool_created_.fetch_add(1, std::memory_order_relaxed);
+    }
+    return ReqPtr(r);
+  }
+  void recycle(Req* r) {
+    if (!pool_open_.load(std::memory_order_acquire)) {
+      delete r;
+      return;
+    }
+    r->body = nullptr;
+    Req* old = free_head_.load(std::memory_order_relaxed);
+    do {
+      r->pool_next.store(old, std::memory_order_relaxed);
+    } while (!free_head_.compare_exchange_weak(old, r, std::memory_order_release, std::memory_order_relaxed));
+  }
+  void free_pool() {
+    pool_open_.store(false, std::memory_order_seq_cst);
+    while (pop_busy_.test_and_set(std::memory_order_acquire)) __builtin_ia32_pause();
+    Req* r = free_head_.exchange(nullptr, std::memory_order_acquire);
+    pop_busy_.clear(std::memory_order_release);
+    while (r) {
+      Req* n = r->pool_next.load(std::memory_order_relaxed);
+      delete r;
+      r = n;
+    }
+  }
+  void pool_counts(int64_t* created, int64_t* reused) const {
+    *created = pool_created_.load(std::memory_order_relaxed);
+    *reused = pool_reused_.load(std::memory_order_relaxed);
+  }
 
   int prepare(Prepared& p, ReqSpec& q, PtrRanges* pr = nullptr) {
     if (q.ndim < 0 || q.ndim > TIPS_MAX_DIMS) return fail(TIPS_ERR_INVALID_ARG, "bad ndim %d", q.ndim);
     if (q.type == TIPS_REQ_ALLGATHER && q.ndim < 1) return fail(TIPS_ERR_INVALID_ARG, "An empty tensor found");
-    auto r = std::make_shared<Req>();
+    ReqPtr r = take();
     r->body = std::move(q.body);
-    r->name = q.name;
+    r->name.assign(q.name);
     r->name_hash = std::hash<std::string>()(r->name);
     r->type = q.type;
     r->root = q.root;
@@ -354,6 +486,7 @@
     r->in = q.in;
     r->out = q.out;
     r->count = 1;
+    r->shape.clear();
     r->shape.reserve((size_t)std::max(q.ndim, 1));
     for (int d = 0; d < q.ndim; d++) {
       if (q.shape[d] < 0) return fail(TIPS_ERR_INVALID_ARG, "negative dimension");
@@ -386,13 +519,22 @@
       }
       r->handle = tl_next++;
     }
-    thread_local NameMap name_scratch;
-    thread_local HandleMap handle_scratch;
-    name_scratch.emplace(NameKey{r->name_hash, r->name}, r);
-    p.name_node = name_scratch.extract(name_scratch.begin());
+    if (r->name_node) {
+      r->name_node.key().h = r->name_hash;
+      r->name_node.key().s.assign(r->name);
+    } else {
+      thread_local NameMap name_scratch;
+      name_scratch.emplace(NameKey{r->name_hash, r->name}, r.get());
+      r->name_node = name_scratch.extract(name_scratch.begin());
+    }
     if (!q.cb) {
-      handle_scratch.emplace(r->handle, r);
-      p.handle_node = handle_scratch.extract(handle_scratch.begin());
+      if (r->handle_node) {
+        r->handle_node.key() = r->handle;
+      } else {
+        thread_local HandleMap handle_scratch;
+        handle_scratch.emplace(r->handle, r.get());
+        r->handle_node = handle_scratch.extract(handle_scratch.begin());
+      }
     }
     p.r = std::move(r);
     return 0;
@@ -408,15 +550,29 @@
   template <class Lap>
   int admit_prepared(Prepared& p, bool handle_anyway, std::string* why, Lap lap) {
     int code = 0;
+    Req& r = *p.r;
     if (!running_) {
       *why = kNotRunning;
       code = TIPS_ERR_NOT_INITIALIZED;
-    } else if (!by_name_.insert(std::move(p.name_node)).inserted) {
-      *why = "a request named " + p.r->name + " is already pending";
-      code = TIPS_ERR_INVALID_ARG;
+    } else {
+      auto res = by_name_.insert(std::move(r.name_node));
+      if (res.inserted) {
+        r.refs.fetch_add(1, std::memory_order_relaxed);
+        if (by_name_.bucket_count() != name_buckets_) {
+          name_buckets_ = by_name_.bucket_count();
+          name_epoch_++;
+        }
+        r.name_it = res.position;
+        r.name_epoch = name_epoch_;
+      } else {
+        r.name_node = std::move(res.node);
+        *why = "a request named " + r.name + " is already pending";
+        code = TIPS_ERR_INVALID_ARG;
+      }
     }
     lap(1);
-    if (p.handle_node && (code == 0 || handle_anyway)) by_handle_.insert(std::move(p.handle_node));
+    if (!r.cb_only && (code == 0 || handle_anyway) && by_handle_.insert(std::move(r.handle_node)).inserted)
+      r.refs.fetch_add(1, std::memory_order_relaxed);
     lap(2);
     if (code == 0) admit(std::move(p.r));
     return code;
@@ -447,10 +603,10 @@
     int64_t gap = gap_us.load(std::memory_order_relaxed);
     if (gap < 0) gap_us.store(gap = std::max<int64_t>(0, env_i64("TIPS_TEST_ENQUEUE_GAP_US", 0)), std::memory_order_relaxed);
     if (gap > 0) std::this_thread::sleep_for(std::chrono::microseconds(gap));
-    Pending* node = new Pending{std::move(p), nullptr};
+    Req* node = p.r.detach();
     thread_local const int tl_shard = (int)(g_next_shard.fetch_add(1, std::memory_order_relaxed) % kShards);
-    std::atomic<Pending*>& head = shards_[tl_shard].head;
-    Pending* old = head.load(std::memory_order_relaxed);
+    std::atomic<Req*>& head = shards_[tl_shard].head;
+    Req* old = head.load(std::memory_order_relaxed);
     do {
       node->next = old;
     } while (!head.compare_exchange_weak(old, node, std::memory_order_seq_cst, std::memory_order_relaxed));
@@ -466,7 +622,7 @@
   }
 
   void reclaim_after_stop() {
-    std::vector<std::shared_ptr<Req>> orphans;
+    std::vector<ReqPtr> orphans;
     {
       std::lock_guard<AdaptiveMutex> l(m_);
       drain_locked(waiter_stop_ ? &orphans : nullptr);
@@ -483,11 +639,11 @@
     waiter_started_.store(true, std::memory_order_release);
   }
 
-  int drain_locked(std::vector<std::shared_ptr<Req>>* orphans = nullptr) {
-    Pending* heads[kShards];
+  int drain_locked(std::vector<ReqPtr>* orphans = nullptr) {
+    Req* heads[kShards];
     int m = 0;
     for (Shard& sh : shards_)
-      if (Pending* h = sh.head.exchange(nullptr, std::memory_order_seq_cst)) heads[m++] = h;
+      if (Req* h = sh.head.exchange(nullptr, std::memory_order_seq_cst)) heads[m++] = h;
     if (!m) return 0;
     int count = 0;
     int64_t t = adm_prof_ ? steady_ns() : 0;
@@ -497,25 +653,24 @@
       adm_ns_[k] += u - t;
       t = u;
     };
-    Pending* rev[kShards] = {};
+    Req* rev[kShards] = {};
     for (bool more = true; more;) {
       more = false;
       for (int k = 0; k < m; k++)
-        if (Pending* h = heads[k]) {
+        if (Req* h = heads[k]) {
           heads[k] = h->next;
-          __builtin_prefetch(h->p.r.get(), 1);
           h->next = rev[k];
           rev[k] = h;
           more = true;
         }
     }
     lap(0);
+    std::string why;
     for (int k = 0; k < m; k++) {
-      for (Pending* q = rev[k]; q;) {
-        Pending* n = q->next;
-        Prepared& p = q->p;
-        Req& r = *p.r;
-        std::string why;
+      for (Req* q = rev[k]; q;) {
+        Req* n = q->next;
+        Prepared p{ReqPtr::adopt(q)};
+        Req& r = *q;
         if (const int code = admit_prepared(p, true, &why, lap)) {
           r.state = kFailed;
           r.code = code;
@@ -527,7 +682,7 @@
           cv_.notify_all();
         }
         lap(3);
-        delete q;
+        p.r.reset();
         lap(4);
         q = n;
         count++;
@@ -536,7 +691,7 @@
     return count;
   }
 
-  void admit(std::shared_ptr<Req>&& r) {
+  void admit(ReqPtr&& r) {
     expect_.admitted(r->name_hash);
     fresh_.push_back(std::move(r));
   }
@@ -563,13 +718,13 @@
   }
 
   int poll(int64_t h, bool block, bool routed = false) {
-    std::shared_ptr<Req> r;
+    ReqPtr r;
     {
       std::unique_lock<AdaptiveMutex> l(m_);
       drain_locked();
       auto it = by_handle_.find(h);
       if (it == by_handle_.end()) return fail(TIPS_ERR_INVALID_ARG, "unknown request handle %lld", (long long)h);
-      r = it->second;
+      r = ReqPtr(it->second);
       if (r->cb) return fail(TIPS_ERR_INVALID_ARG, "request %s completes through its callback (tips_on_done)", r->name.c_str());
       if (block) cv_.wait(l, [&] { return r->resolved(); });
       if (!r->resolved()) return 0;
@@ -582,12 +737,89 @@
       if (e == hipErrorNotReady) return 0;
       if (e != hipSuccess) rc = fail(TIPS_ERR_HIP, "request %s: %s", r->name.c_str(), hipGetErrorString(e));
     }
-    HandleMap::node_type gone;
     {
       std::lock_guard<AdaptiveMutex> l(m_);
-      gone = release_locked(*r);
+      release_locked(*r);
     }
     return rc;
+  }
+
+  int wait_list(const int64_t* hs, int n) {
+    const bool tr = neg_trace();
+    int64_t tw = tr ? steady_ns() : 0, ph[3] = {};
+    auto lap = [&](int k) {
+      if (!tr) return;
+      const int64_t u = steady_ns();
+      ph[k] = u - tw;
+      tw = u;
+    };
+    struct Refused {
+      int i;
+      std::string why;
+    };
+    std::vector<ReqPtr> rs((size_t)n);
+    std::vector<Refused> refused;
+    {
+      std::unique_lock<AdaptiveMutex> l(m_);
+      drain_locked();
+      for (int i = 0; i < n; i++) {
+        if (hs[i] <= 0) continue;
+        auto it = by_handle_.find(hs[i]);
+        if (it == by_handle_.end() || it->second->listed) {
+          refused.push_back(Refused{i, "unknown request handle " + std::to_string((long long)hs[i])});
+        } else if (it->second->cb) {
+          refused.push_back(Refused{i, "request " + it->second->name + " completes through its callback (tips_on_done)"});
+        } else {
+          it->second->listed = true;
+          rs[(size_t)i] = ReqPtr(it->second);
+        }
+      }
+      size_t k = 0;
+      cv_.wait(l, [&] {
+        while (k < rs.size() && (!rs[k] || rs[k]->resolved())) k++;
+        return k == rs.size();
+      });
+    }
+    lap(0);
+    int rc = 0;
+    std::string first;
+    size_t nr = 0;
+    for (int i = 0; i < n; i++) {
+      if (nr < refused.size() && refused[nr].i == i) {
+        if (rc == 0) {
+          rc = TIPS_ERR_INVALID_ARG;
+          first = refused[nr].why;
+        }
+        nr++;
+        continue;
+      }
+      Req* r = rs[(size_t)i].get();
+      if (!r) continue;
+      if (r->state == kFailed) {
+        if (rc == 0) {
+          rc = r->code;
+          first = r->err;
+        }
+      } else if (r->state == kLaunched && !event_done(*r)) {
+        const hipError_t e = finish_event(*r, true);
+        if (e != hipSuccess && rc == 0) {
+          rc = TIPS_ERR_HIP;
+          first = "request " + r->name + ": " + hipGetErrorString(e);
+        }
+      }
+    }
+    lap(1);
+    {
+      std::lock_guard<AdaptiveMutex> l(m_);
+      for (auto& r : rs)
+        if (r) release_locked(*r);
+    }
+    rs.clear();
+    lap(2);
+    if (tr)
+      fprintf(stderr, "[tips neg] wait_n %d handles: blocked %.1f us, event %.1f us, release %.1f us\n", n, ph[0] / 1e3,
+              ph[1] / 1e3, ph[2] / 1e3);
+    return rc ? fail(rc, "%s", first.c_str()) : 0;
   }
 
   static bool event_done(const Req& r) { return r.gev && r.gev->done.load(std::memory_order_acquire); }
@@ -598,11 +830,16 @@
     return e;
   }
 
-  HandleMap::node_type release_locked(Req& r) {
+  void release_locked(Req& r) {
     if (r.ev) ev_pool_.push_back(r.ev);
     r.ev = nullptr;
     r.gev.reset();
-    return r.cb_only ? HandleMap::node_type() : by_handle_.extract(r.handle);
+    r.listed = false;
+    if (r.cb_only) return;
+    auto it = by_handle_.find(r.handle);
+    if (it == by_handle_.end() || it->second != &r) return;
+    r.handle_node = by_handle_.extract(it);
+    ReqPtr::adopt(&r).reset();
   }
 
   int on_done(int64_t h, tips_done_fn fn, void* ctx) {
@@ -610,7 +847,7 @@
     drain_locked();
     auto it = by_handle_.find(h);
     if (it == by_handle_.end()) return fail(TIPS_ERR_INVALID_ARG, "unknown request handle %lld", (long long)h);
-    auto& r = it->second;
+    Req* r = it->second;
     if (r->cb) return fail(TIPS_ERR_INVALID_ARG, "request %s already has a completion callback", r->name.c_str());
     if (waiter_stop_) {
       fn(ctx, r->state == kFailed ? r->code : 0, r->state == kFailed ? r->err.c_str() : "");
@@ -619,7 +856,7 @@
     r->cb = fn;
     r->cb_ctx = ctx;
     start_waiter_locked();
-    if (r->resolved()) queue_done(r);
+    if (r->resolved()) queue_done(ReqPtr(r));
     return 0;
   }
 
@@ -642,6 +879,7 @@
     close_all();
     peers_.clear();
     release_device_resources();
+    free_pool();
     return loop_err_.empty() ? 0 : fail(TIPS_ERR_BOOTSTRAP, "%s", loop_err_.c_str());
   }
 
@@ -671,16 +909,29 @@
       done_cv_.notify_all();
     }
     if (waiter_.joinable()) waiter_.join();
-    std::vector<std::shared_ptr<Req>> orphans;
+    std::vector<ReqPtr> orphans;
     {
       std::lock_guard<AdaptiveMutex> l(m_);
       running_ = false;
       drain_locked(&orphans);
     }
     for (auto& r : orphans) r->cb(r->cb_ctx, r->code, r->err.c_str());
+    orphans.clear();
     for (auto& kv : by_handle_)
-      if (kv.second->ev) ev_pool_.push_back(kv.second->ev);
+      if (kv.second->ev) {
+        ev_pool_.push_back(kv.second->ev);
+        kv.second->ev = nullptr;
+      }
     release_device_resources();
+    free_pool();
+    fresh_.clear();
+    done_q_.clear();
+    exec_req_.reset();
+    waiter_req_.reset();
+    for (auto& kv : by_name_) ReqPtr::adopt(kv.second).reset();
+    by_name_.clear();
+    for (auto& kv : by_handle_) ReqPtr::adopt(kv.second).reset();
+    by_handle_.clear();
   }
 
   bool running() {
@@ -720,8 +971,8 @@
     std::vector<uint32_t> cids;
     std::vector<Req*> full;
     ResponseCache& cache = own_->cache;
+    std::vector<ReqPtr> batch;
     while (true) {
-      std::vector<std::shared_ptr<Req>> batch;
       bool stopping;
       set_phase("waiting for requests");
       long long t_linger = 0, t_tail = 0;
@@ -771,8 +1022,7 @@
           }
         }
         timed_drain();
-        batch.assign(fresh_.begin(), fresh_.end());
-        fresh_.clear();
+        batch.swap(fresh_);
         if (expect_on) {
           for (auto& r : batch) expect_.roll_add(r->name, r->name_hash);
           expect_.roll();
@@ -790,18 +1040,28 @@
           r->classify = false;
         }
       const auto t_x = std::chrono::steady_clock::now();
+      const int64_t ph0 = steady_ns();
       w.b.clear();
       cids.clear();
       full.clear();
       for (auto& r : batch) {
         const int32_t id = cache.cached_id(r->name, r->name_hash, r->type, r->dtype, r->shape, !r->bad.empty());
-        if (id >= 0) cids.push_back((uint32_t)id);
-        else full.push_back(r.get());
+        r->cid = id;
+        if (id >= 0) {
+          cids.push_back((uint32_t)id);
+          if (id_req_.size() <= (size_t)id) id_req_.resize(cache.entries.size(), nullptr);
+          id_req_[(size_t)id] = r.get();
+        } else {
+          full.push_back(r.get());
+        }
       }
       put_announce_head(w, stopping, (uint32_t)full.size());
       for (Req* r : full) put_announce_record(w, r->type, r->root, !r->bad.empty(), r->dtype, r->count, r->shape, r->name);
       put_announce_ids(w, cids);
-      set_phase("exchange (cycle " + std::to_string((long long)cycles_) + ", announcing " + std::to_string(batch.size()) + ")");
+      const size_t nbatch = batch.size();
+      batch.clear();
+      const int64_t ph1 = steady_ns();
+      set_phase("exchange (cycle " + std::to_string((long long)cycles_) + ", announcing " + std::to_string(nbatch) + ")");
       if (!exchange(w.b, &resp)) break;
       {
         std::lock_guard<std::mutex> l(phase_mu_);
@@ -810,7 +1070,9 @@
       bool shutdown = false;
       size_t nd = 0;
       int64_t ncached = 0;
-      const bool wellformed = get_response(resp, cache, &shutdown, ds, &nd, &ncached);
+      const int64_t ph2 = steady_ns();
+      const bool wellformed = get_response(resp, cache, &shutdown, ds, &nd, &ncached, false);
+      const int64_t ph3 = steady_ns();
       cached_decisions_.fetch_add(ncached, std::memory_order_relaxed);
       if (!wellformed) {
         set_loop_error("negotiation: malformed response");
@@ -819,13 +1081,17 @@
       const long long t_exchange = us_since(t_x);
       const auto t_e = std::chrono::steady_clock::now();
       execute(ds, nd);
-      if (trace && (!batch.empty() || nd))
+      if (trace && (nbatch || nd))
         fprintf(stderr, "[tips neg] rank %d cycle %lld: announced %zu, decided %zu; linger %lld us (%d windows, "
                 "ended %lld us after the latest arrival; waits %lld us, admissions %lld us, the last %d in %lld us), exchange %lld us "
-                "(rank 0's decision %lld us), execute %lld us\n", rank_, (long long)cycles_, batch.size(), nd, t_linger, windows,
+                "(rank 0's decision %lld us), execute %lld us\n", rank_, (long long)cycles_, nbatch, nd, t_linger, windows,
                 t_tail, (long long)(wait_ns / 1000), (long long)(drain_ns / 1000), last_drained, (long long)(last_drain_ns / 1000),
                 t_exchange, (long long)(rank_ == 0 ? own_->decide_ns / 1000 : -1), us_since(t_e));
-      if (trace && (!batch.empty() || nd)) {
+      if (trace && (nbatch || nd))
+        fprintf(stderr, "[tips neg]   cycle phases (us): announce %.1f, exchange %.1f, get_response %.1f; execute: lookup %.1f, "
+                "note %.1f, run %.1f, publish %.1f\n", (ph1 - ph0) / 1e3, (ph2 - ph1) / 1e3, (ph3 - ph2) / 1e3, exec_ns_[0] / 1e3,
+                exec_ns_[1] / 1e3, exec_ns_[2] / 1e3, exec_ns_[3] / 1e3);
+      if (trace && (nbatch || nd)) {
         std::lock_guard<AdaptiveMutex> l(m_);
         fprintf(stderr, "[tips neg]   admission phases (us): walk %lld, name table %lld, handle table %lld, queue %lld, "
                 "free %lld\n", (long long)(adm_ns_[0] / 1000), (long long)(adm_ns_[1] / 1000), (long long)(adm_ns_[2] / 1000),
@@ -838,22 +1104,28 @@
     accepting_.store(false, std::memory_order_seq_cst);
     drain_locked();
     running_ = false;
-    std::vector<std::string> unmatched;
-    for (auto& kv : by_name_) unmatched.push_back(kv.first.s);
-    std::sort(unmatched.begin(), unmatched.end());
-    for (auto& name : unmatched) {
-      auto& r = by_name_.find(NameKey{std::hash<std::string>()(name), name})->second;
+    batch.clear();
+    std::vector<Req*> unmatched;
+    for (auto& kv : by_name_) unmatched.push_back(kv.second);
+    std::sort(unmatched.begin(), unmatched.end(), [](const Req* a, const Req* b) { return a->name < b->name; });
+    for (Req* r : unmatched) {
       r->state = kFailed;
       r->code = TIPS_ERR_MISMATCH;
-      r->err = "request " + name + " was not enqueued on every rank before shutdown";
-      if (dry_) log_.push_back(name + " ERR " + r->err);
-      if (r->cb) queue_done(r);
-    }
-    by_name_.clear();
+      r->err = "request " + r->name + " was not enqueued on every rank before shutdown";
+      if (dry_) log_.push_back(r->name + " ERR " + r->err);
+      if (r->cb) queue_done(ReqPtr(r));
+    }
+    for (auto it = by_name_.begin(); it != by_name_.end();) {
+      Req* r = it->second;
+      auto here = it++;
+      r->name_node = by_name_.extract(here);
+      ReqPtr::adopt(r).reset();
+    }
+    std::fill(id_req_.begin(), id_req_.end(), nullptr);
     cv_.notify_all();
   }
 
-  void queue_done(const std::shared_ptr<Req>& r) {
+  void queue_done(const ReqPtr& r) {
     if (r->cb_queued) return;
     r->cb_queued = true;
     done_q_.push_back(r);
@@ -861,7 +1133,7 @@
   }
 
   void waiter_loop() {
-    std::deque<std::shared_ptr<Req>> batch;
+    std::deque<ReqPtr> batch;
     while (true) {
       {
         std::unique_lock<AdaptiveMutex> l(m_);
@@ -886,15 +1158,12 @@
         set_waiter_req(r, false);
         r->cb(r->cb_ctx, status, msg.c_str());
       }
-      set_waiter_req(nullptr, false);
-      std::vector<HandleMap::node_type> gone;
-      gone.reserve(batch.size());
+      set_waiter_req(ReqPtr(), false);
       {
         std::lock_guard<AdaptiveMutex> l(m_);
-        for (auto& r : batch) gone.push_back(release_locked(*r));
+        for (auto& r : batch) release_locked(*r);
         cb_called_ += (int64_t)batch.size();
       }
-      gone.clear();
       batch.clear();
     }
   }
@@ -933,34 +1202,55 @@
   }
 
   void execute(const std::vector<Decision>& ds, size_t n) {
-    std::vector<std::shared_ptr<Req>> reqs(n);
-    std::vector<NameMap::node_type> gone;
-    gone.reserve(n);
+    const bool tr = neg_trace();
+    int64_t te = tr ? steady_ns() : 0;
+    auto lap = [&](int k) {
+      if (!tr) return;
+      const int64_t u = steady_ns();
+      exec_ns_[k] = u - te;
+      te = u;
+    };
+    ResponseCache& cache = own_->cache;
+    std::vector<ReqPtr> reqs(n);
     {
       std::lock_guard<AdaptiveMutex> l(m_);
       for (size_t i = 0; i < n; i++) {
-        look_.h = std::hash<std::string>()(ds[i].name);
-        look_.s.assign(ds[i].name);
-        auto it = by_name_.find(look_);
-        if (it == by_name_.end()) continue;
-        reqs[i] = it->second;
-        gone.push_back(by_name_.extract(it));
+        const Decision& d = ds[i];
+        Req* r = d.id >= 0 && (size_t)d.id < id_req_.size() ? id_req_[(size_t)d.id] : nullptr;
+        NameMap::iterator it;
+        if (r && r->name_epoch == name_epoch_) {
+          it = r->name_it;
+        } else {
+          const std::string& name = r ? r->name : d.id >= 0 ? cache.entries[(size_t)d.id].name : d.name;
+          look_.h = std::hash<std::string>()(name);
+          look_.s.assign(name);
+          it = by_name_.find(look_);
+          if (it == by_name_.end()) continue;
+          r = it->second;
+        }
+        if (r->cid >= 0 && (size_t)r->cid < id_req_.size() && id_req_[(size_t)r->cid] == r) id_req_[(size_t)r->cid] = nullptr;
+        r->name_node = by_name_.extract(it);
+        reqs[i] = ReqPtr::adopt(r);
         if (dry_) {
           std::string sz;
-          for (size_t k = 0; k < ds[i].sizes.size(); k++) sz += (k ? "," : " sizes=") + std::to_string(ds[i].sizes[k]);
-          log_.push_back(ds[i].name + (ds[i].ok ? " OK" + sz : " ERR " + ds[i].err));
-        }
-      }
-    }
-    gone.clear();
+          for (size_t k = 0; k < d.sizes.size(); k++) sz += (k ? "," : " sizes=") + std::to_string(d.sizes[k]);
+          log_.push_back(r->name + (d.ok ? " OK" + sz : " ERR " + d.err));
+        }
+      }
+    }
+    lap(0);
     for (size_t i = 0; i < n; i++) {
-      if (const Req* r = reqs[i].get()) {
+      const Req* r = reqs[i].get();
+      if (ds[i].id >= 0) {
+        if (!r) cache.drop((uint32_t)ds[i].id);
+      } else if (r) {
         const ReqParams rp{r->type, r->dtype, r->count, r->shape};
-        own_->cache.note(ds[i], &rp);
+        cache.note(ds[i], &rp);
       } else {
-        own_->cache.note(ds[i], nullptr);
-      }
-    }
+        cache.note(ds[i], nullptr);
+      }
+    }
+    lap(1);
     std::vector<int> state(n, 0), code(n, TIPS_ERR_MISMATCH);
     std::vector<std::string> msg(n);
     for (size_t i = 0; i < n; i++) {
@@ -1052,6 +1342,11 @@
         i = j;
       }
     }
+    if (!dry_) {
+      std::lock_guard<std::mutex> l(phase_mu_);
+      exec_req_.reset();
+    }
+    lap(2);
     std::lock_guard<AdaptiveMutex> l(m_);
     for (size_t i = 0; i < n; i++)
       if (reqs[i]) {
@@ -1059,8 +1354,10 @@
         reqs[i]->code = code[i];
         reqs[i]->err = msg[i];
         if (reqs[i]->cb) queue_done(reqs[i]);
+        reqs[i].reset();
       }
     cv_.notify_all();
+    lap(3);
   }
 
   int take_event(Req& r) {
@@ -1114,7 +1411,7 @@
     return 0;
   }
 
-  int run_batch(State& st, std::vector<std::shared_ptr<Req>>& reqs, size_t i, size_t j) {
+  int run_batch(State& st, std::vector<ReqPtr>& reqs, size_t i, size_t j) {
     std::vector<hipStream_t> streams;
     for (size_t k = i; k < j; k++)
       if (std::find(streams.begin(), streams.end(), reqs[k]->stream) == streams.end()) streams.push_back(reqs[k]->stream);
@@ -1159,13 +1456,9 @@
   std::condition_variable_any cv_;
   bool running_ = false, want_stop_ = false;
   std::atomic<bool> accepting_{false};
-  struct Pending {
-    Prepared p;
-    Pending* next = nullptr;
-  };
   static constexpr int kShards = 8;
   struct alignas(64) Shard {
-    std::atomic<Pending*> head{nullptr};
+    std::atomic<Req*> head{nullptr};
   };
   Shard shards_[kShards];
   bool any_pending() {
@@ -1176,10 +1469,18 @@
   std::atomic<bool> idle_{false};
   bool lockfree_ = true;
   std::atomic<bool> waiter_started_{false};
-  std::deque<std::shared_ptr<Req>> fresh_;
+  std::atomic<Req*> free_head_{nullptr};
+  std::atomic_flag pop_busy_ = ATOMIC_FLAG_INIT;
+  std::atomic<bool> pool_open_{true};
+  std::atomic<int64_t> pool_created_{0}, pool_reused_{0};
+  std::vector<ReqPtr> fresh_;
   ExpectSet expect_;
   bool adm_prof_ = false;
   int64_t adm_ns_[5] = {};
+  int64_t exec_ns_[4] = {};
+  size_t name_buckets_ = 0;
+  uint64_t name_epoch_ = 1;
+  std::vector<Req*> id_req_;
   std::atomic<int64_t> last_arrival_ns_{0};
   NameMap by_name_;
   NameKey look_{0, std::string()};
@@ -1191,7 +1492,7 @@
   hipStream_t neg_stream_ = nullptr;
   std::thread waiter_;
   int start_cpu_ = -1;
-  std::deque<std::shared_ptr<Req>> done_q_;
+  std::deque<ReqPtr> done_q_;
   std::condition_variable_any done_cv_;
   bool waiter_stop_ = false;
   int64_t cb_called_ = 0;
@@ -1200,17 +1501,17 @@
 
   std::mutex phase_mu_;
   std::string phase_ = "start";
-  std::shared_ptr<Req> waiter_req_;
+  ReqPtr waiter_req_;
   bool waiter_syncing_ = false;
   int64_t cycles_ = 0, executed_ = 0;
   size_t exec_i_ = 0, exec_n_ = 0;
-  std::shared_ptr<Req> exec_req_;
+  ReqPtr exec_req_;
   void set_phase(std::string p) {
     std::lock_guard<std::mutex> l(phase_mu_);
     phase_ = std::move(p);
     exec_req_.reset();
   }
-  void set_waiter_req(const std::shared_ptr<Req>& r, bool syncing) {
+  void set_waiter_req(const ReqPtr& r, bool syncing) {
     std::lock_guard<std::mutex> l(phase_mu_);
     waiter_req_ = r;
     waiter_syncing_ = syncing;
@@ -1249,6 +1550,8 @@
     return out;
   }
 };
+
+void req_unreferenced(Req* r) { r->owner->recycle(r); }
 
 AdaptiveMutex g_neg_mu;
 std::shared_ptr<Negotiator> g_neg;
@@ -1428,6 +1731,7 @@
   };
   int code = TIPS_ERR_NOT_INITIALIZED;
   std::shared_ptr<Negotiator> neg;
+  const int64_t tq0 = neg_trace() ? steady_ns() : 0;
   std::vector<Negotiator::Prepared> ps((size_t)n);
   PtrRanges pr;
   for (int i = 0; i < n; i++) {
@@ -1442,6 +1746,7 @@
     }
     if (e) refused(i, e);
   }
+  const int64_t tq1 = neg_trace() ? steady_ns() : 0;
   if (neg && env_i64("TIPS_LIST_ONE_LOCK", 1) == 0) {
     std::vector<Negotiator::Prepared> one(1);
     for (int i = 0; i < n; i++) {
@@ -1462,6 +1767,9 @@
       first_err = err;
     }
   }
+  if (neg_trace())
+    fprintf(stderr, "[tips neg] enqueue_n %d requests: prepare %.1f us, commit %.1f us\n", n, (tq1 - tq0) / 1e3,
+            (steady_ns() - tq1) / 1e3);
   return rc ? fail(rc, "%s", first_err.c_str()) : 0;
 }
 
@@ -1566,17 +1874,12 @@
 
 int tips_wait_n(const int64_t* handles, int n) {
   if (n < 0 || (n > 0 && !handles)) return fail(TIPS_ERR_INVALID_ARG, "bad handle list");
-  int rc = 0;
-  std::string first_err;
-  for (int i = 0; i < n; i++) {
-    if (handles[i] <= 0) continue;
-    const int w = tips_wait(handles[i]);
-    if (w < 0 && rc == 0) {
-      rc = w;
-      first_err = last_error();
-    }
-  }
-  return rc ? fail(rc, "%s", first_err.c_str()) : 0;
+  bool any = false;
+  for (int i = 0; i < n && !any; i++) any = handles[i] > 0;
+  if (!any) return 0;
+  Negotiator* ng = started();
+  if (!ng) return TIPS_ERR_NOT_INITIALIZED;
+  return ng->wait_list(handles, n);
 }
 
 #ifdef TIPS_DEV
@@ -1584,12 +1887,15 @@
 
 struct SelftestCount {
   std::atomic<int64_t> done{0};
+  std::atomic<bool> hold{false};
 };
 
 void selftest_done(void* ctx, int status, const char* message) {
   (void)status;
   (void)message;
-  static_cast<SelftestCount*>(ctx)->done++;
+  SelftestCount* c = static_cast<SelftestCount*>(ctx);
+  while (c->hold.load()) std::this_thread::sleep_for(std::chrono::milliseconds(1));
+  c->done++;
 }
 
 }
@@ -1635,16 +1941,19 @@
   const auto t0 = std::chrono::steady_clock::now();
   std::vector<SelftestCount> counts(per.size());
   std::vector<int> issued(per.size(), 0), rcs(per.size(), 0);
+  std::atomic<int64_t> cb_requests{0};
   auto run = [&](size_t k) {
-    std::vector<int64_t> handles;
+    std::vector<int64_t> handles, released;
     bool batching = false;
+    bool own_cb = cbs;
+    bool cb_next = false;
     std::vector<Negotiator::Prepared> batch;
     auto issued_one = [&](int64_t h) -> bool {
       if (h < 0) {
         rcs[k] = (int)h;
         return false;
       }
-      if (cbs) {
+      if (own_cb) {
         issued[k]++;
         if (neg.on_done(h, selftest_done, &counts[k]) != 0) {
           rcs[k] = TIPS_ERR_INVALID_ARG;
@@ -1674,12 +1983,48 @@
       } else if (line.rfind("@sleep ", 0) == 0) {
         std::this_thread::sleep_for(std::chrono::milliseconds(atoi(line.c_str() + 7)));
       } else if (line == "@wait") {
-        if (cbs) {
+        if (own_cb) {
           while (counts[k].done.load() < issued[k]) std::this_thread::sleep_for(std::chrono::milliseconds(1));
         } else {
           for (int64_t h : handles) (void)neg.poll(h, true);
           handles.clear();
         }
+      } else if (line == "@handles") {
+        own_cb = false;
+      } else if (line == "@waitn") {
+        const int rc = neg.wait_list(handles.data(), (int)handles.size());
+        neg.note("# waitn rc=" + std::to_string(rc) + (rc ? std::string(" ") + last_error() : std::string()));
+        released.swap(handles);
+        handles.clear();
+      } else if (line == "@pad") {
+        handles.insert(handles.begin(), {(int64_t)0, (int64_t)1 << 60});
+      } else if (line == "@ondone") {
+        if (handles.empty() || neg.on_done(handles.back(), selftest_done, &counts[k]) != 0) {
+          rcs[k] = TIPS_ERR_INVALID_ARG;
+          return;
+        }
+        issued[k]++;
+        cb_requests++;
+      } else if (line == "@hold" || line == "@release") {
+        counts[k].hold.store(line == "@hold");
+      } else if (line == "@cb") {
+        cb_next = true;
+      } else if (line == "@waitcb") {
+        while (counts[k].done.load() < issued[k]) std::this_thread::sleep_for(std::chrono::milliseconds(1));
+      } else if (line == "@stale") {
+        int64_t h = 0;
+        for (int64_t x : released)
+          if (x > 0 && x != (int64_t)1 << 60 && !h) h = x;
+        const int rc = neg.poll(h, true);
+        neg.note("# stale rc=" + std::to_string(rc) + (rc < 0 ? std::string(" ") + last_error() : std::string()));
+      } else if (line == "@state") {
+        neg.note("# state " + neg.debug_state());
+      } else if (line == "@pool") {
+        int64_t made = 0, reused = 0;
+        neg.pool_counts(&made, &reused);
+        neg.note("# pool created " + std::to_string((long long)made) + " reused " + std::to_string((long long)reused));
+      } else if (line == "@stop") {
+        (void)neg.stop();
       } else if (line == "@mark") {
         const auto us = std::chrono::duration_cast<std::chrono::microseconds>(std::chrono::steady_clock::now() - t0);
         neg.note("# mark " + std::to_string((long long)us.count()));
@@ -1689,6 +2034,7 @@
         const int type = strncmp(kind, "ag", 2) == 0 ? TIPS_REQ_ALLGATHER : strncmp(kind, "bc", 2) == 0 ? TIPS_REQ_BROADCAST
                                                                                                     : TIPS_REQ_ALLREDUCE;
         const int root = (type == TIPS_REQ_BROADCAST && kind[2] == ':') ? atoi(kind + 3) : 0;
+        const bool raw_type = strncmp(kind, "ty:", 3) == 0;
         for (const char* q = dims; *q;) {
           shape.push_back(strtoll(q, nullptr, 10));
           q = strchr(q, ',');
@@ -1696,9 +2042,19 @@
         }
         if (shape.empty()) shape.push_back(cnt);
         ReqSpec q(nm, shape.data(), (int)shape.size(), (int)dt);
-        q.type = type;
+        q.type = raw_type ? atoi(kind + 3) : type;
         q.root = root;
-        if (batching) {
+        if (cb_next) {
+          cb_next = false;
+          q.cb = selftest_done;
+          q.cb_ctx = &counts[k];
+          if (neg.enqueue(q) < 0) {
+            rcs[k] = TIPS_ERR_INVALID_ARG;
+            return;
+          }
+          issued[k]++;
+          cb_requests++;
+        } else if (batching) {
           batch.emplace_back();
           if (neg.prepare(batch.back(), q) != 0) {
             rcs[k] = TIPS_ERR_INVALID_ARG;
@@ -1709,7 +2065,7 @@
         }
       }
     }
-    if (!cbs)
+    if (!own_cb)
       for (int64_t h : handles) (void)neg.poll(h, false);
   };
   std::vector<std::thread> threads;
@@ -1722,7 +2078,7 @@
   std::string log;
   for (auto& l : neg.log()) log += l + "\n";
   log += "# cached decisions " + std::to_string((long long)neg.cached_decisions()) + "\n";
-  if (cbs) {
+  if (cbs || cb_requests.load()) {
     int64_t n = 0;
     for (auto& c : counts) n += c.done.load();
     log += "callbacks " + std::to_string((long long)n) + "\n";
```

Result: slower. 6164 (-1.9%).
